# CompVis/stable-diffusion

Measured on AMD Instinct MI355X. Metric: 512x512 images/sec, SD-v1-4 50-step PLMS CFG=7.5, higher is better.
Workload: dtype f16

## Files before the change

### include/sdmi.h

```cpp
#ifndef SDMI_H_
#define SDMI_H_

#include <stdint.h>

#ifdef __cplusplus
extern "C" {
#endif

#define SDMI_ABI_VERSION 17

typedef struct sdmi_unet sdmi_unet;

typedef struct sdmi_unet_cfg {
  int32_t in_channels;
  int32_t out_channels;
  int32_t model_channels;
  int32_t num_res_blocks;
  int32_t n_levels;
  int32_t channel_mult[8];
  int32_t n_attention_resolutions;
  int32_t attention_resolutions[8];
  int32_t num_heads;
  int32_t transformer_depth;
  int32_t context_dim;
// ... 8 lines not shown
#define SDMI_PRECISION_FULL 1
int sdmi_unet_create_with_precision(const sdmi_unet_cfg* cfg, int precision, sdmi_unet** out);
int sdmi_unet_precision(const sdmi_unet* h);
typedef struct sdmi_unet_ext {
  int32_t attention_block;
  int32_t resblock_updown;
} sdmi_unet_ext;
int sdmi_unet_create_ext(const sdmi_unet_cfg* cfg, const sdmi_unet_ext* ext, int precision, sdmi_unet** out);
#define SDMI_UNET_SCALE_SHIFT_NORM 1u
#define SDMI_UNET_NUM_HEAD_CHANNELS_SHIFT 16
#define SDMI_UNET_NUM_HEAD_CHANNELS_MASK 0x0fff0000u
#define SDMI_UNET_NUM_HEAD_CHANNELS(n) (((unsigned)(n) << SDMI_UNET_NUM_HEAD_CHANNELS_SHIFT) & SDMI_UNET_NUM_HEAD_CHANNELS_MASK)
int sdmi_unet_create_flags(const sdmi_unet_cfg* cfg, const sdmi_unet_ext* ext, unsigned flags, int precision, sdmi_unet** out);
int sdmi_unet_destroy(sdmi_unet* h);
int sdmi_unet_num_weights(const sdmi_unet* h);
int sdmi_unet_weight_info(const sdmi_unet* h, int idx, char* key_buf, int key_buf_len, int64_t* shape4, int* ndim);
int sdmi_unet_set_weight(sdmi_unet* h, const char* key, const float* ptr, const int64_t* shape, int ndim, void* stream);
int sdmi_unet_finalize(sdmi_unet* h);

int64_t sdmi_unet_packed_bytes(sdmi_unet* h);
int sdmi_unet_export_packed(sdmi_unet* h, void* host_buf, int64_t bytes, void* stream);
int sdmi_unet_import_packed(sdmi_unet* h, const void* host_buf, int64_t bytes, void* stream);

int64_t sdmi_unet_workspace_bytes(sdmi_unet* h, int B, int H, int W, int Lctx);

int sdmi_unet_cache_context(sdmi_unet* h, const float* ctx, int B, int Lctx, void* workspace, int64_t workspace_bytes,
                            void* stream);
int sdmi_unet_reserve_context(sdmi_unet* h, int B, int Lctx);

int sdmi_unet_cache_timesteps(sdmi_unet* h, const int64_t* t_host, int n, void* stream);
int sdmi_unet_hint_timestep(sdmi_unet* h, int64_t t);
int sdmi_unet_tape_stats(sdmi_unet* h, int64_t* replayed, int64_t* recorded);
int sdmi_unet_skip_fold_plan(sdmi_unet* h, int B, int H, int W, int Lctx, int32_t* folded, int cap);

int sdmi_unet_forward(sdmi_unet* h, const float* x, const int64_t* t_i64, const float* t_f32, const float* ctx,
                      float* eps_out, int B, int H, int W, int Lctx, void* workspace, int64_t workspace_bytes,
                      void* stream);

int sdmi_sampler_step(const float* eps_model, int cfg, float scale, const float* x, int mode, const float* old0,
                      const float* old1, const float* old2, float a_t, float a_prev, float sigma, float sqrt_1m_at,
                      const float* noise, float* e_t_out, float* x_prev, float* pred_x0, int64_t n, void* stream);

int sdmi_sampler_step_x0(const float* eps_model, int cfg, float scale, const float* x, int mode, const float* old0, const float* old1,
                         const float* old2, float a_t, float sqrt_1m_at, float* e_t_out, float* ep_out, float* pred_x0, int64_t n,
                         void* stream);
int sdmi_sampler_step_from_x0(const float* pred_x0, const float* ep, float a_prev, float sigma, const float* noise, float* x_prev,
                              int64_t n, void* stream);

int sdmi_ddpm_step(const float* eps, const float* x0_in, const float* x, float c_recip, float c_recipm1, int clip, float coef1,
                   float coef2, float s, const float* noise, const float* mask, const float* x0_orig, const float* q_noise, float sa,
                   float s1ma, float* x0_out, float* x_prev, int64_t n, void* stream);


int sdmi_dpm_solver_step(const float* eps_model, int cfg, float scale, const float* x, const float* m_prev, float alpha_s,
                         float sigma_s, float cx, float a, float inv_r0, int order, float* m_out, float* x_next, int64_t n,
                         void* stream);

typedef struct sdmi_vae sdmi_vae;
typedef struct sdmi_vae_cfg {
  int32_t ch;
  int32_t out_ch;
  int32_t n_levels;
  int32_t ch_mult[8];
  int32_t num_res_blocks;
  int32_t in_channels;
  int32_t z_channels;
// ... 124 lines not shown

typedef struct sdmi_igemm_desc {
  const void* a0; const void* a1; const void* a2;
  int32_t c0, c1, c2, lda0, lda1, lda2;
  int32_t B, Hin, Win, Hout, Wout, ksize, stride, up;
  const void* w;
  int32_t N;
  int32_t mode;
  const float* bias; const float* rowvec; int32_t ld_rowvec;
  const float* residual; int32_t ldr;
  float* out_f32; void* out_f16; int32_t ldo;
  void* seg_dst[3]; int32_t seg_kind[3];
  int32_t heads, dh, ntok, ntok_pad, segC;
  int32_t splitk;
  float* splitk_ws; int64_t splitk_ws_floats;
  int32_t tile;
  int32_t dma;
  int32_t asym_pad;
  int32_t gn_n; void* gn_acc[2]; int32_t gn_cpg[2]; int32_t gn_cbase[2];
  int32_t* splitk_cnt; int32_t splitk_cnt_ints;
  int32_t split16;
  const float* f16_scale; float* lnp_out;
  const float* lnf_part; int32_t lnf_npart; float lnf_eps; const float* lnf_cs; const float* lnf_d;
  const float* pgn_gamma; const float* pgn_beta; float pgn_eps; int32_t pgn_silu;
  void* pgn_out; int32_t pgn_keep_f32; int32_t* pgn_applied;
  void* out_lo;
} sdmi_igemm_desc;
int sdmi_k_igemm(const sdmi_igemm_desc* d, void* stream);
int sdmi_k_igemm_tail(const sdmi_igemm_desc* d, const void* t0, const void* t1, const void* t2, int tail_c, int tail_ld, const void* tail_w,
                      int tail_kt, void* stream);
int sdmi_k_tail_split_range(int nkt, int nsplit, int split, int* begin, int* end);
int sdmi_k_igemm_up_phase(const sdmi_igemm_desc* d, void* stream);
int sdmi_k_up_phase_weights(const void* w_packed_f16, void* dst_f16, int N, int Cin, void* stream);
int sdmi_k_ff_tail(const sdmi_igemm_desc* proj_out, const void* ln_f16, const float* lnp, float ln_eps, const float* csd,
                   const void* wgg_f16, const void* wff2_f16, const float* bff2, const float* t, void* stream);
int sdmi_k_st_tail(const sdmi_igemm_desc* proj_out, const void* a_f16, const void* wo_f16, const float* bo, float* t, const float* ln_gamma,
                   float ln_eps, const float* csd, const void* wgg_f16, const void* wff2_f16, const float* bff2, void* stream);
int sdmi_k_gn_conv3(const sdmi_igemm_desc* conv, const float* x0, const float* x1, int c0, int c1, float* gn_ws, int64_t gn_ws_floats,
                    const float* gn_gamma, const float* gn_beta, float gn_eps, void* stream);
int sdmi_k_st_head(const float* x, float* gn_ws, int64_t gn_ws_floats, const float* gn_gamma, const float* gn_beta, float gn_eps,
                   const void* w_in3, const float* b_in, float* t, const float* ln_gamma, float ln_eps, const void* wqkv_f16,
                   const float* lnf_cs, const float* lnf_d, void* q, void* k, void* vt, int B, int ntok, int ntok_pad, int heads, int dh,
                   int C, void* stream);
int sdmi_k_st_mid(const void* a_f16, const void* wo_f16, const float* bo, float* t, const float* ln_gamma, float ln_eps, const void* wq_f16,
                  const float* lnf_cs, const float* lnf_d, void* q, int B, int ntok, int heads, int dh, int C, void* stream);
int sdmi_k_st_mid_ctx(const void* a_f16, const void* wo_f16, const float* bo, float* t, const float* ln_gamma, float ln_eps, const void* wq_f16,
                      const float* lnf_cs, const float* lnf_d, const void* ctx_k, const void* ctx_vt, int nkv, int nkv_pad, float scale, void* ao_out,
                      int B, int ntok, int heads, int dh, int C, void* stream);
int sdmi_k_ln_fold_prep(const void* w_f16, int N, int K, int ldw, const float* gamma, const float* beta, const float* bias,
                        float* cs, float* d, void* stream);
int sdmi_k_attention(const void* q, const void* k, const void* vt, void* out, int BH, int heads, int nq, int nkv,
                     int nkv_pad, int d, float scale, void* stream);
int sdmi_k_attention_split16(const void* q, const void* q_lo, const void* k, const void* k_lo, const void* vt, const void* vt_lo, void* out,
                             void* out_lo, int BH, int heads, int nq, int nkv, int nkv_pad, int d, float scale, void* stream);
int sdmi_k_attention_split16_causal(const void* q, const void* q_lo, const void* k, const void* k_lo, const void* vt, const void* vt_lo,
                                    void* out, void* out_lo, int BH, int heads, int n, int n_pad, int d, float scale, void* stream);
int sdmi_k_attention_causal(const void* q, const void* k, const void* vt, void* out, int BH, int heads, int n, int n_pad,
                            int d, float scale, void* stream);
int sdmi_k_groupnorm(const float* x0, const float* x1, int c0, int c1, int B, int HW, const float* gamma,
                     const float* beta, float eps, int silu, void* out_f16, float* out_f32, void* raw_f16, void* out_lo,
                     void* raw_lo, float* partial_ws, int64_t partial_floats, void* stream);
int64_t sdmi_k_groupnorm_ws_floats(int B, int HW);
int sdmi_k_groupnorm_film(const float* x0, const float* x1, int c0, int c1, int B, int HW, const float* gamma, const float* beta, float eps,
                          int silu, const float* film, int film_ld, void* out_f16, float* out_f32, void* raw_f16, void* out_lo, void* raw_lo,
                          float* partial_ws, int64_t partial_floats, void* stream);
int sdmi_k_layernorm(const float* x, const float* gamma, const float* beta, void* out_f16, int M, int C, float eps,
// ... 57 lines not shown
```

### stable-diffusion_amd/_lib.py

```python
import ctypes as C
import os

_HERE = os.path.dirname(os.path.abspath(__file__))
LIB_PATH = os.environ.get('SDMI_LIB_PATH') or os.path.join(_HERE, 'libsdmi.so')

c_f32p = C.c_void_p
c_ptr = C.c_void_p


class UNetCfg(C.Structure):
    _fields_ = [('in_channels', C.c_int32), ('out_channels', C.c_int32), ('model_channels', C.c_int32),
                ('num_res_blocks', C.c_int32), ('n_levels', C.c_int32), ('channel_mult', C.c_int32 * 8),
                ('n_attention_resolutions', C.c_int32), ('attention_resolutions', C.c_int32 * 8),
                ('num_heads', C.c_int32), ('transformer_depth', C.c_int32), ('context_dim', C.c_int32)]


class VaeCfg(C.Structure):
    _fields_ = [('ch', C.c_int32), ('out_ch', C.c_int32), ('n_levels', C.c_int32), ('ch_mult', C.c_int32 * 8),
                ('num_res_blocks', C.c_int32), ('in_channels', C.c_int32), ('z_channels', C.c_int32),
                ('embed_dim', C.c_int32)]


class UNetExt(C.Structure):
    _fields_ = [('attention_block', C.c_int32), ('resblock_updown', C.c_int32)]
# ... 122 lines not shown
    'sdmi_vit_create': (C.c_int, [C.POINTER(VitCfg), C.POINTER(c_ptr)]),
    'sdmi_vit_destroy': (C.c_int, [c_ptr]),
    'sdmi_vit_num_weights': (C.c_int, [c_ptr]),
    'sdmi_vit_weight_info': (C.c_int, [c_ptr, C.c_int, C.c_char_p, C.c_int, C.POINTER(C.c_int64), C.POINTER(C.c_int)]),
    'sdmi_vit_set_weight': (C.c_int, [c_ptr, C.c_char_p, c_ptr, C.POINTER(C.c_int64), C.c_int, c_ptr]),
    'sdmi_vit_finalize': (C.c_int, [c_ptr]),
    'sdmi_vit_workspace_bytes': (C.c_int64, [c_ptr, C.c_int]),
    'sdmi_vit_forward': (C.c_int, [c_ptr, c_ptr, c_ptr, c_ptr, c_ptr, C.c_int, c_ptr, C.c_int64, c_ptr]),
    'sdmi_k_vit_kpad': (C.c_int, [C.c_int]),
    'sdmi_k_vit_patchify': (C.c_int, [c_ptr, c_ptr, C.c_int, C.c_int, C.c_int, c_ptr]),
    'sdmi_k_vit_embed': (C.c_int, [c_ptr, c_ptr, c_ptr, c_ptr, C.c_int, C.c_int, C.c_int, c_ptr]),
    'sdmi_k_vit_preprocess': (C.c_int, [c_ptr, c_ptr, C.c_int, C.c_int, C.c_int, C.c_int, c_ptr]),
    'sdmi_k_safety_head': (C.c_int, [c_ptr, c_ptr, c_ptr, c_ptr, c_ptr, c_ptr, c_ptr, c_ptr, C.c_int, C.c_int, C.c_int, C.c_int, c_ptr]),
    'sdmi_knn_create': (C.c_int, [C.c_int, C.c_int64, C.POINTER(c_ptr)]),
    'sdmi_knn_destroy': (C.c_int, [c_ptr]),
    'sdmi_knn_set_rows': (C.c_int, [c_ptr, C.c_int64, C.c_int64, c_ptr, c_ptr]),
    'sdmi_knn_finalize': (C.c_int, [c_ptr, c_ptr]),
    'sdmi_knn_rows': (C.c_int64, [c_ptr]),
    'sdmi_knn_dim': (C.c_int, [c_ptr]),
    'sdmi_knn_workspace_bytes': (C.c_int64, [c_ptr, C.c_int, C.c_int]),
    'sdmi_knn_search': (C.c_int, [c_ptr, c_ptr, C.c_int, C.c_int, c_ptr, c_ptr, c_ptr, c_ptr, C.c_int64, c_ptr]),
    'sdmi_knn_condition': (C.c_int, [c_ptr, c_ptr, C.c_int, C.c_int, c_ptr, c_ptr, c_ptr, c_ptr, C.c_int64, c_ptr]),
    'sdmi_k_knn_inv_norm': (C.c_int, [c_ptr, C.c_int64, C.c_int, c_ptr, c_ptr]),
    'sdmi_k_knn_scan': (C.c_int, [c_ptr, c_ptr, C.c_int64, C.c_int, c_ptr, C.c_int, C.c_int, C.c_int64, c_ptr, c_ptr, c_ptr]),
    'sdmi_k_knn_merge': (C.c_int, [c_ptr, c_ptr, C.c_int, C.c_int, C.c_int, c_ptr, c_ptr, c_ptr]),
    'sdmi_k_knn_stream_read': (C.c_int, [c_ptr, C.c_int64, c_ptr, c_ptr]),
    'sdmi_k_knn_gather': (C.c_int, [c_ptr, c_ptr, C.c_int64, C.c_int, c_ptr, C.c_int, C.c_int, c_ptr, c_ptr, C.c_int64, c_ptr]),
    'sdmi_has_experiments': (C.c_int, []),
    'sdmi_k_igemm': (C.c_int, [C.POINTER(IGemmDesc), c_ptr]),
    'sdmi_k_igemm_tail': (C.c_int, [C.POINTER(IGemmDesc), c_ptr, c_ptr, c_ptr, C.c_int, C.c_int, c_ptr, C.c_int, c_ptr]),
    'sdmi_k_tail_split_range': (C.c_int, [C.c_int, C.c_int, C.c_int, C.POINTER(C.c_int), C.POINTER(C.c_int)]),
    'sdmi_k_igemm_up_phase': (C.c_int, [C.POINTER(IGemmDesc), c_ptr]),
    'sdmi_k_up_phase_weights': (C.c_int, [c_ptr, c_ptr, C.c_int, C.c_int, c_ptr]),
    'sdmi_tune_lookup': (C.c_int, [C.c_int] * 9 + [C.POINTER(C.c_int), C.POINTER(C.c_int)]),
    'sdmi_unet_skip_fold_plan': (C.c_int, [c_ptr, C.c_int, C.c_int, C.c_int, C.c_int, C.POINTER(C.c_int32), C.c_int]),
    'sdmi_k_ff_tail': (C.c_int, [C.POINTER(IGemmDesc), c_ptr, c_ptr, C.c_float, c_ptr, c_ptr, c_ptr, c_ptr, c_ptr, c_ptr]),
    'sdmi_k_gn_conv3': (C.c_int, [C.POINTER(IGemmDesc), c_ptr, c_ptr, C.c_int, C.c_int, c_ptr, C.c_int64, c_ptr, c_ptr, C.c_float, c_ptr]),
    'sdmi_k_st_mid_ctx': (C.c_int, [c_ptr, c_ptr, c_ptr, c_ptr, c_ptr, C.c_float, c_ptr, c_ptr, c_ptr, c_ptr, c_ptr, C.c_int, C.c_int, C.c_float, c_ptr,
                                    C.c_int, C.c_int, C.c_int, C.c_int, C.c_int, c_ptr]),
    'sdmi_k_st_tail': (C.c_int, [C.POINTER(IGemmDesc), c_ptr, c_ptr, c_ptr, c_ptr, c_ptr, C.c_float, c_ptr, c_ptr, c_ptr, c_ptr, c_ptr]),
    'sdmi_k_st_mid': (C.c_int, [c_ptr, c_ptr, c_ptr, c_ptr, c_ptr, C.c_float, c_ptr, c_ptr, c_ptr, c_ptr, C.c_int, C.c_int, C.c_int, C.c_int,
                                C.c_int, c_ptr]),
    'sdmi_k_st_head': (C.c_int, [c_ptr, c_ptr, C.c_int64, c_ptr, c_ptr, C.c_float, c_ptr, c_ptr, c_ptr, c_ptr, C.c_float, c_ptr, c_ptr, c_ptr,
                                 c_ptr, c_ptr, c_ptr, C.c_int, C.c_int, C.c_int, C.c_int, C.c_int, C.c_int, c_ptr]),
    'sdmi_k_attention_split16': (C.c_int, [c_ptr, c_ptr, c_ptr, c_ptr, c_ptr, c_ptr, c_ptr, c_ptr, C.c_int, C.c_int, C.c_int, C.c_int,
                                           C.c_int, C.c_int, C.c_float, c_ptr]),
    'sdmi_k_attention_split16_causal': (C.c_int, [c_ptr, c_ptr, c_ptr, c_ptr, c_ptr, c_ptr, c_ptr, c_ptr, C.c_int, C.c_int, C.c_int, C.c_int,
                                                  C.c_int, C.c_float, c_ptr]),
    'sdmi_k_attention_causal': (C.c_int, [c_ptr, c_ptr, c_ptr, c_ptr, C.c_int, C.c_int, C.c_int, C.c_int, C.c_int, C.c_float,
                                          c_ptr]),
    'sdmi_k_pointwise_nchw': (C.c_int, [c_ptr, c_ptr, c_ptr, c_ptr, C.c_int, C.c_int, C.c_int, C.c_int, C.c_float, c_ptr]),
    'sdmi_k_softmax_rows': (C.c_int, [c_ptr, c_ptr, C.c_int, C.c_int, C.c_float, c_ptr]),
    'sdmi_k_gelu_erf': (C.c_int, [c_ptr, c_ptr, C.c_int64, c_ptr]),
    'sdmi_k_quick_gelu': (C.c_int, [c_ptr, c_ptr, C.c_int64, c_ptr]),
    'sdmi_k_quick_gelu_split': (C.c_int, [c_ptr, c_ptr, c_ptr, C.c_int64, c_ptr]),
    'sdmi_k_gelu_erf_split': (C.c_int, [c_ptr, c_ptr, c_ptr, C.c_int64, c_ptr]),
    'sdmi_k_attention': (C.c_int, [c_ptr, c_ptr, c_ptr, c_ptr, C.c_int, C.c_int, C.c_int, C.c_int, C.c_int, C.c_int,
                                   C.c_float, c_ptr]),
    'sdmi_k_groupnorm': (C.c_int, [c_ptr, c_ptr, C.c_int, C.c_int, C.c_int, C.c_int, c_ptr, c_ptr, C.c_float, C.c_int,
                                   c_ptr, c_ptr, c_ptr, c_ptr, c_ptr, c_ptr, C.c_int64, c_ptr]),
    'sdmi_k_groupnorm_ws_floats': (C.c_int64, [C.c_int, C.c_int]),
    'sdmi_k_groupnorm_film': (C.c_int, [c_ptr, c_ptr, C.c_int, C.c_int, C.c_int, C.c_int, c_ptr, c_ptr, C.c_float, C.c_int, c_ptr, C.c_int,
                                        c_ptr, c_ptr, c_ptr, c_ptr, c_ptr, c_ptr, C.c_int64, c_ptr]),
    'sdmi_k_layernorm': (C.c_int, [c_ptr, c_ptr, c_ptr, c_ptr, C.c_int, C.c_int, C.c_float, c_ptr]),
    'sdmi_k_cast_f16': (C.c_int, [c_ptr, c_ptr, c_ptr, C.c_int64, c_ptr]),
    'sdmi_k_split_heads': (C.c_int, [c_ptr, C.c_int, C.c_int, c_ptr, c_ptr, C.c_int, C.c_int, C.c_int, C.c_int, C.c_int, C.c_int,
# ... 70 lines not shown
```

### stable-diffusion_amd/build.py

```python
import concurrent.futures as cf
import hashlib
import os
import subprocess
import sys

HERE = os.path.dirname(os.path.abspath(__file__))
CSRC = os.path.join(HERE, 'csrc')
EXTRA = os.environ.get('SDMI_CXXFLAGS', '').split()
LIB = os.path.join(HERE, os.environ.get('SDMI_LIB_OUT', 'libsdmi.so'))
OBJ = os.path.join(HERE, 'build' if os.path.basename(LIB) == 'libsdmi.so' else 'build_' + os.path.splitext(os.path.basename(LIB))[0])
SOURCES = ['igemm_t1.hip', 'igemm_t0.hip', 'igemm_t2.hip', 'igemm_h1.hip', 'igemm_h0.hip', 'igemm_h2.hip', 'igemm.hip', 'conv3halo.hip', 'gemm_split16.hip', 'rowchain.hip', 'gnconv.hip', 'range.hip', 'attn.hip', 'attn_wide.hip', 'attn_split16.hip', 'attn_wide_split16.hip', 'split_ops.hip', 'norm.hip', 'small.hip', 'sampler.hip', 'inpaint.hip', 'patch.hip', 'vit.hip', 'knn.hip', 'textpool.hip', 'rescale.hip', 'weights.cpp', 'unet.cpp', 'vae.cpp', 'clip.cpp', 'bert.cpp', 'api.cpp', 'prof.cpp']
FLAGS = ['--offload-arch=gfx950', '-O3', '-std=c++17', '-fPIC', '-munsafe-fp-atomics', '-Wall', '-Wno-unused-function',
         '-Wno-unused-variable']


def _hipcc():
    for c in (os.environ.get('HIPCC'), '/opt/rocm/bin/hipcc', 'hipcc'):
        if c and (not os.path.isabs(c) or os.path.exists(c)):
            return c
    raise RuntimeError('hipcc not found')


def _stamp():
    h = hashlib.sha256()
    for root in (CSRC, os.path.join(os.path.dirname(HERE), 'include')):
        for fn in sorted(os.listdir(root)):
            with open(os.path.join(root, fn), 'rb') as f:
                h.update(fn.encode())
                h.update(f.read())
    h.update(' '.join(FLAGS + EXTRA).encode())
    return h.hexdigest()


def is_current():
    stamp_file = os.path.join(OBJ, 'stamp')
    return os.path.exists(LIB) and os.path.exists(stamp_file) and open(stamp_file).read() == _stamp()


def build(force=False, verbose=True):
    os.makedirs(OBJ, exist_ok=True)
    stamp_file = os.path.join(OBJ, 'stamp')
    if not force and is_current():
        return LIB
    hipcc = _hipcc()
# ... 56 lines not shown
```

### stable-diffusion_amd/csrc/api.cpp

```cpp
#include <string.h>

#include <new>

#include "prof.h"
#include "split16.h"
#include "unet.h"
#include "vae.h"
#include "clip.h"
#include "knn.h"
#include "rescale.h"

namespace sdmi {
static thread_local std::string g_err;
void set_error(const std::string& msg) { g_err = msg; }
int fail(const std::string& msg) { g_err = msg; return -1; }
}

struct sdmi_unet { sdmi::UNet impl; };
struct sdmi_vae { sdmi::Vae impl; };
struct sdmi_clip { sdmi::ClipText impl; };
struct sdmi_bert { sdmi::BertText impl; };
struct sdmi_vit { sdmi::ClipVision impl; };
struct sdmi_knn { sdmi::Knn impl; };

// ... 523 lines not shown
  p.pgn_gamma = d->pgn_gamma; p.pgn_beta = d->pgn_beta; p.pgn_eps = d->pgn_eps; p.pgn_silu = d->pgn_silu;
  p.pgn_out = (f16*)d->pgn_out; p.pgn_keep_f32 = d->pgn_keep_f32; p.pgn_applied = d->pgn_applied;
  p.out_lo = (f16*)d->out_lo;
  return zero_page(&p.zero_page);
}
int sdmi_k_igemm(const sdmi_igemm_desc* d, void* stream) {
  SDMI_CHECK(d, "null descriptor");
  IGemmParams p = IGemmParams();
  if (igemm_params_of(d, p)) return -1;
  IGemmTune t; t.tile = d->tile; t.dma = d->dma;
  return launch_igemm(p, t, (hipStream_t)stream);
}
int sdmi_k_igemm_tail(const sdmi_igemm_desc* d, const void* t0, const void* t1, const void* t2, int tail_c, int tail_ld, const void* tail_w,
                      int tail_kt, void* stream) {
  SDMI_CHECK(d, "null descriptor");
  IGemmParams p = IGemmParams();
  if (igemm_params_of(d, p)) return -1;
  p.tail_a0 = (const f16*)t0; p.tail_a1 = (const f16*)t1; p.tail_a2 = (const f16*)t2;
  p.tail_c = tail_c; p.tail_ld = tail_ld; p.tail_w = (const f16*)tail_w; p.tail_kt = tail_kt;
  IGemmTune t; t.tile = d->tile; t.dma = d->dma;
  return launch_igemm(p, t, (hipStream_t)stream);
}
int sdmi_k_igemm_up_phase(const sdmi_igemm_desc* d, void* stream) {
  SDMI_CHECK(d, "null descriptor");
  IGemmParams p = IGemmParams();
  if (igemm_params_of(d, p)) return -1;
  SDMI_CHECK(p.ksize == 3 && p.up == 1 && p.stride == 1 && p.Hout == 2 * p.Hin && p.Wout == 2 * p.Win && p.c1 == 0 && p.c2 == 0 && !p.split16,
             "up_phase: the descriptor is the reference op, a 3x3 stride-1 conv of one nearest-x2 upsampled source (Hout = 2 Hin, Wout = 2 Win)");
  IGemmParams q = up_phase_of(p, p.w);
  q.splitk = d->splitk;
  IGemmTune t; t.tile = d->tile; t.dma = d->dma;
  return launch_igemm(q, t, (hipStream_t)stream);
}
int sdmi_k_up_phase_weights(const void* w_packed, void* dst, int N, int Cin, void* stream) {
  return launch_up_phase_weights((const f16*)w_packed, (f16*)dst, N, Cin, (hipStream_t)stream);
}
int sdmi_k_tail_split_range(int nkt, int nsplit, int split, int* begin, int* end) {
  SDMI_CHECK(begin && end && nkt >= 0 && nsplit >= 1 && split >= 0 && split < nsplit, "bad arguments");
  tail_split_range(nkt, nsplit, split, begin, end);
  return 0;
}
int sdmi_tune_lookup(int M, int N, int K, int ksize, int stride, int up, int mode, int splitk_req, int kt, int* tile, int* splitk) {
  SDMI_CHECK(tile && splitk, "null argument");
  return tune_lookup(M, N, K, ksize, stride, up, mode, splitk_req, kt, tile, splitk);
}
int sdmi_unet_skip_fold_plan(sdmi_unet* h, int B, int H, int W, int Lctx, int32_t* folded, int cap) {
  SDMI_CHECK(h && (folded || cap == 0), "null argument");
  int64_t need = 0;
  if (h->impl.run(nullptr, nullptr, nullptr, nullptr, nullptr, B, H, W, Lctx, nullptr, 0, nullptr, true, false, &need)) return -1;
  const std::vector<int>& plan = h->impl.skip_fold_plan_;
  for (int i = 0; i < (int)plan.size() && i < cap; ++i) folded[i] = plan[i];
  return (int)plan.size();
}
int sdmi_k_ff_tail(const sdmi_igemm_desc* proj_out, const void* ln_f16, const float* lnp, float ln_eps, const float* csd,
                   const void* wgg_f16, const void* wff2_f16, const float* bff2, const float* t, void* stream) {
  SDMI_CHECK(proj_out, "null descriptor");
  FfTailParams q = FfTailParams();
  if (igemm_params_of(proj_out, q.epi)) return -1;
  SDMI_CHECK(proj_out->split16 && proj_out->ksize == 1, "ff_tail: the proj_out descriptor is a split-fp16 1x1 (w = sdmi_k_pack_split3)");
  q.ln = (const f16*)ln_f16; q.lnp = lnp; q.ln_eps = ln_eps; q.csd = csd; q.wgg = (const f16*)wgg_f16; q.wff2 = (const f16*)wff2_f16;
  q.bff2 = bff2; q.t = t; q.wpo = (const f16*)proj_out->w;
  return launch_ff_tail(q, (hipStream_t)stream);
}
int sdmi_k_st_tail(const sdmi_igemm_desc* proj_out, const void* a_f16, const void* wo_f16, const float* bo, float* t, const float* ln_gamma,
                   float ln_eps, const float* csd, const void* wgg_f16, const void* wff2_f16, const float* bff2, void* stream) {
  SDMI_CHECK(proj_out && a_f16, "null argument");
  FfTailParams q = FfTailParams();
  if (igemm_params_of(proj_out, q.epi)) return -1;
  SDMI_CHECK(proj_out->split16 && proj_out->ksize == 1, "st_tail: the proj_out descriptor is a split-fp16 1x1 (w = sdmi_k_pack_split3)");
  q.a16 = (const f16*)a_f16; q.wo = (const f16*)wo_f16; q.bo = bo; q.ln_gamma = ln_gamma; q.ln_eps = ln_eps; q.csd = csd;
  q.wgg = (const f16*)wgg_f16; q.wff2 = (const f16*)wff2_f16; q.bff2 = bff2; q.t = t; q.wpo = (const f16*)proj_out->w;
  return launch_ff_tail(q, (hipStream_t)stream);
}
int sdmi_k_gn_conv3(const sdmi_igemm_desc* conv, const float* x0, const float* x1, int c0, int c1, float* gn_ws, int64_t gn_ws_floats,
                    const float* gn_gamma, const float* gn_beta, float gn_eps, void* stream) {
  SDMI_CHECK(conv && x0 && gn_ws && gn_gamma && gn_beta, "gn_conv3: null argument");
  GnConvParams q = GnConvParams();
  if (igemm_params_of(conv, q.epi)) return -1;
  const int B = q.epi.B;
  SDMI_CHECK(gn_ws_floats >= gn_acc_words(B) * 2, "groupnorm workspace too small");
  SDMI_HIP_OK(hipMemsetAsync(gn_ws, 0, gn_acc_words(B) * sizeof(long long), (hipStream_t)stream));
  GroupNormParams g = GroupNormParams();
  g.x0 = x0; g.c0 = c0; g.x1 = x1; g.c1 = c1; g.B = B; g.HW = q.epi.Hout * q.epi.Wout; g.gamma = gn_gamma; g.beta = gn_beta; g.eps = gn_eps;
// ... 185 lines not shown
```

### stable-diffusion_amd/csrc/common.h

```cpp
#pragma once
#include <hip/hip_runtime.h>
#include <stdint.h>
#include <algorithm>
#include <string>

#include "tape.h"

typedef _Float16 f16;
typedef _Float16 f16x2 __attribute__((ext_vector_type(2)));
typedef _Float16 f16x4 __attribute__((ext_vector_type(4)));
typedef _Float16 f16x8 __attribute__((ext_vector_type(8)));
typedef float f32x4 __attribute__((ext_vector_type(4)));
typedef float f32x16 __attribute__((ext_vector_type(16)));

#ifdef __HIPCC__
__device__ __forceinline__ float gn_apply_elem(float v, float mean, float rstd, float gamma, float beta, int silu) {
  float t = __builtin_fmaf((v - mean) * rstd, gamma, beta);
  if (silu) t = t * __builtin_amdgcn_rcpf(1.0f + __expf(-t));
  return t;
}
__device__ __forceinline__ float gn_apply_film_elem(float v, float mean, float rstd, float gamma, float beta, float scale, float shift,
                                                    int silu) {
  float t = __builtin_fmaf((v - mean) * rstd, gamma, beta);
  t = __builtin_fmaf(t, 1.0f + scale, shift);
// ... 15 lines not shown
  *hi = (long long)h;
  *lo = __double2ll_rn((d - h) * 1099511627776.0);
}
__device__ __forceinline__ void gn_mean_rstd(long long s, long long sl, long long ss, long long ssl, double n, float eps,
                                             float* mean, float* rstd) {
  const double m = gn_acc_value(s, sl) / n;
  double var = gn_acc_value(ss, ssl) / n - m * m;
  if (var < 0.0) var = 0.0;
  *mean = (float)m;
  *rstd = (float)(1.0 / sqrt(var + (double)eps));
}
#endif

namespace sdmi {

void set_error(const std::string& msg);
int fail(const std::string& msg);

#define SDMI_HIP_OK(expr)                                                                    \
  do {                                                                                       \
    hipError_t _e = (expr);                                                                  \
    if (_e != hipSuccess)                                                                    \
      return ::sdmi::fail(std::string(#expr) + ": " + hipGetErrorString(_e));                \
  } while (0)

#define SDMI_CHECK(cond, msg)                                                                \
  do {                                                                                       \
    if (!(cond)) return ::sdmi::fail(std::string("check failed: ") + #cond + " -- " + (msg)); \
  } while (0)

static inline int cdiv(int a, int b) { return (a + b - 1) / b; }
static inline int64_t round_up(int64_t a, int64_t b) { return (a + b - 1) / b * b; }

enum EpiMode { EPI_PLAIN = 0, EPI_GEGLU = 1, EPI_HEADS = 2 };

#ifdef SDMI_NT_STORES
#define SDMI_ST(T, ptr, val) __builtin_nontemporal_store((T)(val), (T*)(ptr))
#else
#define SDMI_ST(T, ptr, val) (*(T*)(ptr) = (T)(val))
#endif
#ifndef SDMI_W_AUX
#define SDMI_W_AUX 0
#endif
#ifndef SDMI_WT_STORES
#define SDMI_WT_STORES 1
#endif
#if defined(__HIPCC__) && SDMI_WT_STORES >= 1
typedef unsigned sdmi_u32x4 __attribute__((ext_vector_type(4)));
typedef unsigned sdmi_u32x2 __attribute__((ext_vector_type(2)));
__device__ __forceinline__ void sdmi_st_wt16(const void* base, size_t byte_off, f32x4 v) {
  if (__builtin_expect(byte_off < (size_t)0x80000000u - 16, 1)) {
    const __amdgpu_buffer_rsrc_t r = __builtin_amdgcn_make_buffer_rsrc((void*)base, 0, (int)0x80000000, 0x00020000);
    __builtin_amdgcn_raw_buffer_store_b128(__builtin_bit_cast(sdmi_u32x4, v), r, (int)byte_off, 0, 16);
  } else {
    *(f32x4*)((char*)base + byte_off) = v;
  }
}
__device__ __forceinline__ void sdmi_st_wt8(const void* base, size_t byte_off, f16x4 v) {
  if (__builtin_expect(byte_off < (size_t)0x80000000u - 16, 1)) {
    const __amdgpu_buffer_rsrc_t r = __builtin_amdgcn_make_buffer_rsrc((void*)base, 0, (int)0x80000000, 0x00020000);
    __builtin_amdgcn_raw_buffer_store_b64(__builtin_bit_cast(sdmi_u32x2, v), r, (int)byte_off, 0, 16);
  } else {
    *(f16x4*)((char*)base + byte_off) = v;
  }
}
#define SDMI_ST_F32X4(base, off, val) sdmi_st_wt16((base), (size_t)(off) * 4, (val))
#if SDMI_WT_STORES >= 2
// ... 39 lines not shown
  int nkt = 0;
#ifdef SDMI_IGEMM_TIMING
  long long* dbg_times = nullptr;
  int dbg_abl = 0;
#endif
  int splitk_fused = 0;
  int slab_tiled = 0, slab_bm = 0, slab_bn = 0, slab_wm = 0, slab_wn = 0;
  int slab_sh_qpt = 0, slab_sh_nt = 0, slab_sh_tn = 0, slab_sh_wn = 0;
  int epi_vec = 0;
  int tile_n_fastest = 0;
  const f16* zero_page = nullptr;
  int gn_n = 0;
  long long* gn_acc[2] = {nullptr, nullptr};
  int gn_cpg[2] = {0, 0}, gn_cbase[2] = {0, 0};
  unsigned long long gn_magic[2] = {0, 0};
  const float* pgn_gamma = nullptr; const float* pgn_beta = nullptr; float pgn_eps = 1e-5f; int pgn_silu = 1;
  f16* pgn_out = nullptr;
  int pgn_keep_f32 = 0;
  int* pgn_applied = nullptr;
  unsigned long long magic_hw = 0, magic_w = 0, magic_w2 = 0;
  int log2w = 0;
  const float* xf0 = nullptr; const float* xf1 = nullptr;
  const long long* gn_in_acc = nullptr;
  const float* gn_in_gamma = nullptr; const float* gn_in_beta = nullptr; float gn_in_eps = 1e-5f; int gn_in_silu = 1;
  f16* raw_hi = nullptr; f16* raw_lo = nullptr;
  f16* gn_scratch = nullptr;
  unsigned long long magic_cpg_in = 0;
  int halo_thi = 0, halo_ipt = 1, log2_tpi = 30;
  unsigned long long magic_hpi = 0;
  const f16* tail_a0 = nullptr; const f16* tail_a1 = nullptr; const f16* tail_a2 = nullptr;
  int tail_c = 0, tail_ld = 0;
  const f16* tail_w = nullptr;
  int tail_kt = 0;
};
__host__ __device__ static inline void tail_split_range(int nkt, int nsplit, int split, int* begin, int* end) {
  *begin = (int)(((long long)split * nkt) / nsplit);
  *end = (int)(((long long)(split + 1) * nkt) / nsplit);
}

constexpr int SDMI_NUM_TILES = 22;
struct IGemmTune {
  int tile = -1;
  int dma = -1;
};

int launch_igemm(const IGemmParams& p, const IGemmTune& tune, hipStream_t stream);
bool igemm_plans_halo(const IGemmParams& p);
bool igemm_plans_up_phase(const IGemmParams& p);
static inline IGemmParams up_phase_of(const IGemmParams& p, const f16* w_phase) {
  IGemmParams q = p;
  q.ksize = 2; q.Hout = p.Hin; q.Wout = p.Win; q.M = p.B * p.Hin * p.Win; q.K = 4 * p.c0; q.w = w_phase; q.splitk = 0;
  return q;
}
int tune_lookup(int M, int N, int K, int ksize, int stride, int up, int mode, int splitk_req, int kt, int* tile, int* splitk);
bool range_check_enabled();
uint64_t tune_generation();
bool tune_collecting();
int range_check_set(int enable);
int range_scan(const char* what, const f16* p, int64_t n, hipStream_t stream);
int range_report(std::string* json);

int tune_begin();
int tune_round(int r);
int tune_end(const char* path, int* n_keys);
int tune_dump(std::string* out);
int launch_splitk_reduce(const IGemmParams& p, int nsplit, hipStream_t stream);
// ... 40 lines not shown
  long long* dbg = nullptr;
#endif
};
bool st_head_supported(int C, int M, int ntok, int ntok_pad, int heads, int dh);
int launch_st_head(const StHeadParams& p, hipStream_t stream);
int launch_st_mid(const StHeadParams& p, hipStream_t stream);

struct GnConvParams {
  const float* x0 = nullptr; const float* x1 = nullptr; int c0 = 0, c1 = 0;
  const long long* gn_acc = nullptr;
  const float* gn_gamma = nullptr; const float* gn_beta = nullptr; float gn_eps = 1e-5f;
  const f16* w = nullptr;
#ifdef SDMI_RC_TIMING
  long long* dbg = nullptr;
#endif
  IGemmParams epi;
};
bool gn_conv3_supported(int B, int H, int W, int c0, int c1, int Cout);
int launch_gn_conv3(const GnConvParams& p, hipStream_t stream);

struct AttnParams {
  const f16* q = nullptr;
  const f16* k = nullptr;
  const f16* vt = nullptr;
  f16* out = nullptr;
  int BH = 0, heads = 0, nq = 0, nkv = 0, nkv_pad = 0, d = 0;
  float scale = 1.f;
  int nw = 0;
  int causal = 0;
  int prio = 0;
  int pingpong = 0;
};
int launch_attention(const AttnParams& p, hipStream_t stream);
int launch_attention_wide(const AttnParams& p, hipStream_t stream);

struct GroupNormParams {
  const float* x0 = nullptr; const float* x1 = nullptr; int c0 = 0, c1 = 0;
  int B = 0, HW = 0;
  const float* gamma = nullptr; const float* beta = nullptr; float eps = 1e-5f;
  int silu = 0;
  int stats_only = 0;
  int skip_stats = 0;
  f16* out_f16 = nullptr;
  float* out_f32 = nullptr;
  f16* raw_f16 = nullptr;
  f16* out_lo = nullptr;
  f16* raw_lo = nullptr;
  const float* film = nullptr; int film_ld = 0;
  long long* acc = nullptr;
};
constexpr int GN_SLOTS = 8;
constexpr int GN_MAX_CALLS = 96;
constexpr int GN_WORDS = 4;
constexpr int GN_STRIDE = 16;
static inline int64_t gn_acc_words(int B) { return (int64_t)B * 32 * GN_SLOTS * GN_STRIDE; }
int launch_groupnorm(const GroupNormParams& p, hipStream_t stream);

int launch_layernorm(const float* x, const float* gamma, const float* beta, f16* out, int M, int C, float eps,
                     hipStream_t stream, float* out_f32 = nullptr);
int launch_cast_f16(const float* x, f16* out, f16* out_lo, int64_t n, hipStream_t stream);

int launch_timestep_embedding(const int64_t* t_i64, const float* t_f32, float* out, int B, int dim, hipStream_t s);
int launch_small_linear(const float* in, int ld_in, const float* w, const float* bias, float* out, int ld_out,
                        int B, int N, int K, int silu_in, hipStream_t s);
int launch_ctx1_broadcast(const f16* vt, int ld_v, f16* ao, int B, int ntok, int C, hipStream_t s);
int launch_conv_in(const float* x_nchw, const float* w, const float* bias, float* out_nhwc, int B, int Cin, int H,
// ... 98 lines not shown
```

### stable-diffusion_amd/csrc/igemm.hip

```cpp
#include <dlfcn.h>

#include <map>
#include <mutex>
#include <tuple>
#include <vector>

#include "igemm_dev.h"

namespace sdmi {
namespace {

__global__ void __launch_bounds__(256) splitk_reduce_kernel(IGemmParams p, int nsplit, int rows_per_block) {
  __shared__ unsigned long long s_gn[2][32][GN_WORDS];
  const int tx = threadIdx.x & 7, ty = threadIdx.x >> 3;
  const int n = (blockIdx.x * 8 + tx) * 4;
  const int row0 = blockIdx.y * rows_per_block;
  const int HW = p.Hout * p.Wout;
  const bool gn = p.gn_n > 0;
  const bool ncol = n < p.N;
  if (gn) {
    for (int i = threadIdx.x; i < 2 * 32 * GN_WORDS; i += 256) (&s_gn[0][0][0])[i] = 0ull;
    __syncthreads();
  }
  const size_t slab_sz = (size_t)p.M * p.N;
// ... 343 lines not shown
  SDMI_HIP_OK(hipGetLastError());
  ps2.end();
  if (p.ln_out) return launch_layernorm(p.out_f32, p.ln_gamma, p.ln_beta, p.ln_out, p.M, p.N, p.ln_eps, stream);
  return 0;
}

struct TileCfg { int bm, bn, wm, wn, ns; };
static const TileCfg kTiles[SDMI_NUM_TILES] = {
    {128, 128, 2, 2, 2},
    {128, 64, 2, 2, 2},
    {64, 64, 2, 2, 2},
    {256, 128, 4, 2, 2},
    {128, 64, 2, 2, 3},
    {64, 64, 2, 2, 3},
    {256, 128, 4, 2, 3},
    {128, 128, 2, 2, 3},
    {64, 128, 2, 2, 3},
    {128, 128, 4, 2, 3},
    {64, 64, 2, 2, 4},
    {128, 256, 2, 4, 2},
    {64, 256, 1, 4, 3},
    {256, 64, 4, 1, 3},
    {256, 64, 4, 2, 5},
    {256, 128, 4, 2, 3},
    {128, 64, 2, 2, 8},
    {128, 128, 2, 2, 5},
    {64, 64, 2, 2, 8},
    {64, 128, 2, 2, 6},
    {128, 64, 2, 2, 6},
    {128, 128, 4, 2, 4},
};
static inline bool tile_is_halo(int t) { return t >= 14 && t <= 17; }
static inline bool tile_tn_even(int t) { return (kTiles[t].bn / kTiles[t].wn / 32) % 2 == 0; }

static int launch_tile(int tile, const IGemmParams& p, bool dma, int splitk, hipStream_t stream) {
  if (p.tail_kt && !tile_is_halo(tile)) return fail("a GEMM with a 1x1 tail phase was routed to tile " + std::to_string(tile) + ": only the halo-staged conv tiles 14..17 run a tail");
  if (p.split16) return launch_split16_tile(tile, p, splitk, stream);
  if (igemm_has_half(p)) {
    switch (tile) {
      case 0: case 1: case 2: case 3: case 4: case 5: return launch_generic_tile_h0(tile, p, dma, splitk, stream);
      case 6: case 7: case 8: case 9: case 10: return launch_generic_tile_h1(tile, p, dma, splitk, stream);
      case 11: case 12: case 13: case 18: case 19: case 20: case 21: return launch_generic_tile_h2(tile, p, dma, splitk, stream);
      default: break;
    }
  }
  switch (tile) {
    case 0: case 1: case 2: case 3: case 4: case 5: return launch_generic_tile_g0(tile, p, dma, splitk, stream);
    case 6: case 7: case 8: case 9: case 10: return launch_generic_tile_g1(tile, p, dma, splitk, stream);
    case 11: case 12: case 13: case 18: case 19: case 20: case 21: return launch_generic_tile_g2(tile, p, dma, splitk, stream);
    case 14: case 15: case 16: case 17: return launch_halo_tile(tile, p, splitk, stream);
    default: return fail("unknown igemm tile id");
  }
}

struct TuneKey {
  int M, N, K, ksize, stride, up, mode, splitk_req;
  int kt = 0;
  bool operator<(const TuneKey& o) const {
    return std::tie(M, N, K, ksize, stride, up, mode, splitk_req, kt) <
           std::tie(o.M, o.N, o.K, o.ksize, o.stride, o.up, o.mode, o.splitk_req, o.kt);
  }
};
struct TuneChoice { int tile, splitk; double us; };
struct TuneRec { TuneKey key; int cand; hipEvent_t e0, e1; };

class Tuner {
 public:
  std::mutex mu;
  std::map<TuneKey, TuneChoice> table;
  bool loaded = false, collecting = false;
  int round = 0;
  std::vector<TuneRec> recs;
  std::map<TuneKey, std::vector<std::pair<TuneChoice, std::vector<float>>>> stats;
  std::vector<hipEvent_t> pool;

  static std::string default_path() {
    if (const char* e = getenv("SDMI_TUNE_FILE")) return e;
    Dl_info info;
    if (dladdr((const void*)&Tuner::default_path, &info) && info.dli_fname) {
      std::string so = info.dli_fname;
      const size_t k = so.find_last_of('/');
      return (k == std::string::npos ? std::string(".") : so.substr(0, k)) + "/tune_gfx950.txt";
    }
    return "tune_gfx950.txt";
  }
  static std::string phase_path_of(const std::string& table_path) {
    static const std::string base = "tune_gfx950.txt";
    if (table_path.size() >= base.size() && table_path.compare(table_path.size() - base.size(), base.size(), base) == 0)
      return table_path.substr(0, table_path.size() - base.size()) + "tune_up_phase_gfx950.txt";
    return table_path + ".up_phase";
  }
  void load_file(const std::string& path) {
    FILE* f = fopen(path.c_str(), "r");
    if (!f) return;
    char line[256];
    while (fgets(line, sizeof line, f)) {
      if (line[0] == '#') continue;
      TuneKey k; TuneChoice c; c.us = 0;
      k.kt = 0;
      if (sscanf(line, "%d %d %d %d %d %d %d %d %d %d %lf %d", &k.M, &k.N, &k.K, &k.ksize, &k.stride, &k.up, &k.mode,
                 &k.splitk_req, &c.tile, &c.splitk, &c.us, &k.kt) >= 10 && c.tile >= 0 && c.tile < SDMI_NUM_TILES && c.splitk >= 1 &&
          c.splitk <= 16 && k.kt >= 0)
        table[k] = c;
    }
    fclose(f);
  }
  void ensure_loaded() {
    if (loaded) return;
    loaded = true;
    if (env_int("SDMI_TUNE_DISABLE", 0)) return;
    load_file(default_path());
    load_file(phase_path_of(default_path()));
  }
  std::map<TuneKey, TuneChoice>::const_iterator find_entry(TuneKey k) const {
    auto it = table.find(k);
    if (it == table.end() && k.kt) { k.kt = 0; it = table.find(k); }
    return it;
  }
  hipEvent_t ev() {
    if (!pool.empty()) { hipEvent_t e = pool.back(); pool.pop_back(); return e; }
    hipEvent_t e = nullptr;
    (void)hipEventCreate(&e);
    return e;
  }
};
static Tuner g_tuner;

static std::vector<TuneChoice> tune_candidates(const IGemmParams& p, bool can_split) {
  std::vector<TuneChoice> out;
  const int nkt = igemm_nkt(p);
  static const int splits[] = {1, 2, 3, 4, 5, 6, 8, 10, 12, 16};
  for (int t = 0; t < SDMI_NUM_TILES; ++t) {
    const TileCfg& c = kTiles[t];
    if (tile_is_halo(t) && !halo_supported(p, c.bm)) continue;
    if (p.tail_kt && !tile_is_halo(t)) continue;
    if (p.split16 && !split16_tile_supported(t)) continue;
    if (!p.split16 && ((c.ns == 2 && t != 11 && !tile_is_halo(t)) || t == 12 || t == 13)) continue;
    if (p.mode == EPI_GEGLU && !tile_tn_even(t)) continue;
    if (p.lnp_out && (p.M % c.bm || p.N % c.bn || (p.Hout * p.Wout) % c.bm)) continue;
    const long blocks = (long)cdiv(p.M, c.bm) * cdiv(p.N, c.bn);
    if ((long)c.bm > 2L * p.M && c.bm > 64) continue;
    if ((long)c.bn > 2L * p.N && c.bn > 64) continue;
    for (int sk : splits) {
      if ((sk == 5 || sk == 10) && !tile_is_halo(t)) continue;
      if (sk > 1) {
        if (p.splitk != 0 || !can_split || p.ksize == 2) break;
        if (nkt / sk < 4) break;
        if (tile_is_halo(t) && (nkt / 9) % sk != 0) continue;
        if (blocks * (sk / 2 + 1) > 1536) break;
        if (splitk_ws_need(p, c.bm, c.bn, sk) > p.splitk_ws_floats) break;
      }
      if (blocks * sk < 48 && sk < 16 && nkt / (sk * 2) >= 4 && can_split && p.splitk == 0 && p.ksize != 2) continue;
      out.push_back({t, p.splitk > 1 ? p.splitk : sk, 0.0});
      if (p.splitk != 0) break;
    }
  }
  if (out.empty()) out.push_back({5, p.splitk > 0 ? p.splitk : 1, 0.0});
  return out;
}

int tune_begin() {
  std::lock_guard<std::mutex> lk(g_tuner.mu);
  g_tuner.ensure_loaded();
  g_tuner.collecting = true; g_tuner.round = 0;
  g_tuner.recs.clear(); g_tuner.stats.clear();
  return 0;
}
int tune_round(int r) {
  std::lock_guard<std::mutex> lk(g_tuner.mu);
  g_tuner.round = r;
  return 0;
}
static int tune_drain() {
  for (auto& r : g_tuner.recs) {
    float ms = 0.f;
    SDMI_HIP_OK(hipEventSynchronize(r.e1));
    SDMI_HIP_OK(hipEventElapsedTime(&ms, r.e0, r.e1));
    auto& v = g_tuner.stats[r.key];
    if ((int)v.size() > r.cand) v[r.cand].second.push_back(ms * 1e3f);
    g_tuner.pool.push_back(r.e0); g_tuner.pool.push_back(r.e1);
  }
  g_tuner.recs.clear();
  return 0;
}
bool tune_collecting() { return g_tuner.collecting; }
static uint64_t g_tune_generation = 0;
uint64_t tune_generation() { return g_tune_generation; }
int tune_end(const char* path, int* n_keys) {
  std::lock_guard<std::mutex> lk(g_tuner.mu);
  if (!g_tuner.collecting) return fail("sdmi_tune_end without sdmi_tune_begin");
  if (tune_drain()) return -1;
  g_tuner.collecting = false;
  auto score = [](std::vector<float> v) -> double {
    if (v.empty()) return 1e30;
    std::sort(v.begin(), v.end());
    return v.size() % 2 ? v[v.size() / 2] : 0.5 * (v[v.size() / 2 - 1] + v[v.size() / 2]);
  };
  for (auto& kv : g_tuner.stats) {
    double best = 1e30; const TuneChoice* bc = nullptr;
    for (auto& c : kv.second) {
      const double sc = score(c.second);
      if (sc < best) { best = sc; bc = &c.first; }
    }
    if (bc) g_tuner.table[kv.first] = {bc->tile, bc->splitk, best};
  }
  if (n_keys) *n_keys = (int)g_tuner.stats.size();
  ++g_tune_generation;
  const std::string out = (path && *path) ? std::string(path) : Tuner::default_path();
  bool any_phase = false;
  for (auto& kv : g_tuner.table) any_phase = any_phase || kv.first.ksize == 2;
  for (int which = 0; which < (any_phase ? 2 : 1); ++which) {
    const std::string path_w = which ? Tuner::phase_path_of(out) : out;
    FILE* f = fopen(path_w.c_str(), "w");
    if (!f) return fail("cannot write the tuning table to " + path_w);
    fputs(which ? "# libsdmi igemm tuning table (gfx950), the 2x2 phase convs of the Upsample convs (ksize 2: M = rows of one phase, K = 4 Cin; compared with "
                       "the site's up = 1 row of the main table), measured in situ by tools/tune.py -- M N K ksize stride up mode splitk_req tile splitk us\n"
                     : "# libsdmi igemm tuning table (gfx950), measured in situ by tools/tune.py -- M N K ksize stride up mode splitk_req tile splitk us\n", f);
    for (auto& kv : g_tuner.table) {
      const TuneKey& k = kv.first;
      if ((k.ksize == 2) != (which == 1)) continue;
      fprintf(f, "%d %d %d %d %d %d %d %d %d %d %.2f", k.M, k.N, k.K, k.ksize, k.stride, k.up, k.mode, k.splitk_req, kv.second.tile,
              kv.second.splitk, kv.second.us);
      if (k.kt) fprintf(f, " %d", k.kt);
      fprintf(f, "\n");
    }
    fclose(f);
  }
  return 0;
}
int tune_dump(std::string* out) {
  std::lock_guard<std::mutex> lk(g_tuner.mu);
  char buf[256];
  for (auto& kv : g_tuner.stats) {
    const TuneKey& k = kv.first;
    for (auto& c : kv.second) {
      if (c.second.empty()) continue;
      std::vector<float> v = c.second;
      std::sort(v.begin(), v.end());
      snprintf(buf, sizeof buf, "%d %d %d %d %d %d %d %d%s | %d %d %.2f %.2f %d\n", k.M, k.N, k.K, k.ksize, k.stride, k.up, k.mode,
               k.splitk_req, k.kt ? (" t" + std::to_string(k.kt)).c_str() : "", c.first.tile, c.first.splitk, (double)v[v.size() / 2], (double)v[0], (int)v.size());
      *out += buf;
    }
  }
  return 0;
}

int tune_lookup(int M, int N, int K, int ksize, int stride, int up, int mode, int splitk_req, int kt, int* tile, int* splitk) {
  std::lock_guard<std::mutex> lk(g_tuner.mu);
  g_tuner.ensure_loaded();
  auto it = g_tuner.find_entry(TuneKey{M, N, K, ksize, stride, up, mode, splitk_req, kt});
  if (it == g_tuner.table.end()) return 1;
  *tile = it->second.tile; *splitk = it->second.splitk;
  return 0;
// ... 44 lines not shown
               "upsample phase convs: nearest x2 of one source of whole 64-channel chunks (Hout x Wout = the SOURCE map), plain epilogue without residual / "
               "LayerNorm / tail, unsplit");
  const int Cin = p.c0 + p.c1 + p.c2;
  SDMI_CHECK(p.K == p.ksize * p.ksize * Cin, "K != ksize^2 * (c0 + c1 + c2)");
  SDMI_CHECK(p.c0 % BKH == 0 && p.c1 % BKH == 0 && p.c2 % BKH == 0 && p.c0 > 0, "channel counts of every A source must be multiples of 32");
  SDMI_CHECK((p.c2 == 0 || p.c1 > 0), "third A source without a second");
  SDMI_CHECK(p.lda0 % 8 == 0 && (p.a1 == nullptr || p.lda1 % 8 == 0), "A row pitch must be a multiple of 8 halves");
  SDMI_CHECK(p.zero_page != nullptr, "zero page missing");
  SDMI_CHECK(p.M == p.B * p.Hout * p.Wout, "M != B * Hout * Wout");
  SDMI_CHECK(p.c1 == 0 || p.a1 != nullptr, "second A source missing");
  SDMI_CHECK(p.c2 == 0 || (p.a2 != nullptr && p.lda2 % 8 == 0), "third A source missing");
  SDMI_CHECK((p.c1 == 0 || p.lda1 == p.lda0) && (p.c2 == 0 || p.lda2 == p.lda0), "all A sources must share one row pitch");
  SDMI_CHECK(!p.up || ((p.ksize == 3 || phase) && p.stride == 1), "upsample folding needs a 3x3 stride-1 conv");
  if (p.mode == EPI_GEGLU) SDMI_CHECK(p.N % 64 == 0 && p.out_f16 != nullptr, "GEGLU needs N % 64 == 0 and an fp16 output");
  if (p.ln_out)
    SDMI_CHECK(p.mode == EPI_PLAIN && p.out_f32 && p.ldo == p.N && p.N % 4 == 0 && p.N <= 2560 && p.ln_gamma && p.ln_beta,
               "LayerNorm post-op needs plain mode, an fp32 output with ldo == N <= 2560, gamma and beta");
  if (p.out_lo) SDMI_CHECK(p.mode == EPI_PLAIN && p.ldo % 4 == 0, "out_lo needs plain mode");
  if (p.lnp_out || p.f16_scale)
    SDMI_CHECK(p.mode == EPI_PLAIN && p.out_f32 && p.out_f16 && !p.out_lo && !p.ln_out && p.N % 64 == 0 && p.M % 64 == 0 &&
                   (p.Hout * p.Wout) % 64 == 0 && p.splitk == 1 && epi_vec_ok(p),
               "LayerNorm row statistics: plain mode, fp32 + fp16 outputs, no split-K, M / N / rows per sample multiples of 64, 16-byte aligned rows");
  if (p.lnf_part)
    SDMI_CHECK(p.ksize == 1 && p.c1 == 0 && p.c2 == 0 && !p.split16 && p.lnf_npart * 32 == p.K && p.lnf_cs && p.lnf_d && !p.bias &&
                   p.splitk == 1 && p.lnf_npart <= 40,
               "LayerNorm-folding GEMM: dense, one source, K = 32 * lnf_npart <= 1280, column sums + offsets, no bias, no split-K");
  if (p.gn_n) {
    SDMI_CHECK(p.mode == EPI_PLAIN && p.gn_n <= 2 && (p.Hout * p.Wout) % 32 == 0, "GroupNorm statistics need plain mode and Hout*Wout % 32 == 0");
    SDMI_CHECK(p.N % 4 == 0, "GroupNorm statistics: N % 4 == 0");
    for (int t = 0; t < p.gn_n; ++t)
      SDMI_CHECK(p.gn_acc[t] && p.gn_cpg[t] >= 2 && (p.gn_cbase[t] + p.N + p.gn_cpg[t] - 1) / p.gn_cpg[t] <= 32, "bad GroupNorm statistics target");
  }
  if (p.mode == EPI_HEADS) SDMI_CHECK(p.segC > 0 && p.dh > 0 && p.N % p.segC == 0 && p.N / p.segC <= 3, "bad head scatter");

  SDMI_CHECK((int64_t)p.B * p.Hin * p.Win * p.lda0 * 2 + (int64_t)(p.Win + 1) * p.lda0 * 2 < ((int64_t)1 << 31) - 65536 &&
                 (int64_t)p.N * p.K * 2 < ((int64_t)1 << 31) - 65536,
             "tensor too large for 31-bit byte offsets (buffer addressing)");
  static const int env_dma = env_int("SDMI_IGEMM_DMA", 1);
  static const int env_tile = env_int("SDMI_IGEMM_TILE", -1);
  const bool dma = (tune.dma >= 0 ? tune.dma : env_dma) != 0;
  int tile = tune.tile >= 0 ? tune.tile : env_tile;
  SDMI_CHECK(tile < SDMI_NUM_TILES, "unknown igemm tile id");
  int splitk = p.splitk;
  const int nkt = igemm_nkt(p);
  static const int env_split = env_int("SDMI_SPLITK", -1);
  const bool can_split_plain = p.mode == EPI_PLAIN && p.splitk_ws && p.N % 4 == 0 && p.ldo % 4 == 0 &&
                               (p.residual == nullptr || p.ldr % 4 == 0);
  const bool can_split_heads = p.mode == EPI_HEADS && p.splitk_ws && p.dh % 4 == 0 && p.segC % 4 == 0;
  const bool can_split = can_split_plain || can_split_heads;
  if (env_split >= 0 && splitk == 0 && !phase) splitk = env_split;

  hipEvent_t ev0 = nullptr, ev1 = nullptr;
  TuneKey tkey{p.M, p.N, nkt * BK, p.split16 ? 11 : p.ksize, p.stride, p.up, p.mode, splitk, p.tail_kt};
  int tcand = -1;
  if (tile < 0) {
    std::lock_guard<std::mutex> lk(g_tuner.mu);
    g_tuner.ensure_loaded();
    static const int only_ksize = env_int("SDMI_TUNE_ONLY_KSIZE", -1);
    if (g_tuner.collecting && (only_ksize < 0 || tkey.ksize == only_ksize)) {
      IGemmParams q = p; q.splitk = splitk;
      const std::vector<TuneChoice> cands = tune_candidates(q, can_split);
      auto& st = g_tuner.stats[tkey];
      if (st.empty()) for (auto& c : cands) st.push_back({c, {}});
      tcand = g_tuner.round % (int)cands.size();
      tile = cands[tcand].tile; splitk = cands[tcand].splitk;
      ev0 = g_tuner.ev(); ev1 = g_tuner.ev();
    } else {
      auto it = g_tuner.find_entry(tkey);
      if (it != g_tuner.table.end()) {
        const int tt = it->second.tile, sk = it->second.splitk;
        const bool halo = tile_is_halo(tt);
        const bool ws_ok = sk == 1 || (can_split && splitk_ws_need(p, kTiles[tt].bm, kTiles[tt].bn, sk) <= p.splitk_ws_floats);
        const bool split_ok = splitk != 0 ? (sk == splitk && ws_ok)
                                          : (sk == 1 || (ws_ok && nkt / sk >= 4 && (halo || (sk != 5 && sk != 10)) &&
                                                         (!halo || (nkt / 9) % sk == 0)));
        if (split_ok && (p.mode != EPI_GEGLU || tile_tn_even(tt)) && (!halo || halo_supported(p, kTiles[tt].bm)) &&
            (!p.split16 || split16_tile_supported(tt)) && (!phase || sk == 1)) {
          tile = tt; splitk = sk;
        }
      }
    }
  }
  if (p.mode == EPI_GEGLU && tile >= 0 && !tile_tn_even(tile)) tile = 0;
  if (p.split16) {
    if (tile >= 0) SDMI_CHECK(split16_tile_supported(tile), "split-fp16 GEMM: tile id without an instantiation");
    else tile = 5;
  }
  if (tile < 0) {
    const double gflop = 2.0 * p.M * (double)p.N * p.K * 1e-9;
    if (p.mode == EPI_GEGLU) tile = 0;
    else if (p.mode == EPI_HEADS) tile = 2;
    else tile = gflop >= 25.0 ? 3 : 5;
  }
  if (p.lnp_out) {
    const int hw = p.Hout * p.Wout;
    if (p.M % kTiles[tile].bm || p.N % kTiles[tile].bn || hw % kTiles[tile].bm || (p.split16 && !split16_tile_supported(tile))) tile = 5;
  }
  if (phase) {
    SDMI_CHECK(!tile_is_halo(tile) && splitk <= 1, "upsample phase convs run unsplit on the generic tiles");
    splitk = 1;
  }
  if (splitk <= 0) {
    splitk = 1;
    if (can_split) {
      const long blocks = (long)cdiv(p.M, kTiles[tile].bm) * cdiv(p.N, kTiles[tile].bn);
      const long want = (kTiles[tile].wm * kTiles[tile].wn == 8) ? 160 : 512;
      while (blocks * splitk < want && nkt / (splitk * 2) >= 8 && splitk < 16 &&
             splitk_ws_need(p, kTiles[tile].bm, kTiles[tile].bn, splitk * 2) <= p.splitk_ws_floats)
        splitk *= 2;
    }
  }
  if (splitk > 1) {
    SDMI_CHECK(can_split, "split-K needs plain or head-scatter mode, a slab workspace and N / ldo / ldr multiples of 4");
    SDMI_CHECK(splitk_ws_need(p, kTiles[tile].bm, kTiles[tile].bn, splitk) <= p.splitk_ws_floats, "split-K workspace too small");
  }
  if (ev0) SDMI_HIP_OK(hipEventRecord(ev0, stream));
#ifdef SDMI_IGEMM_TIMING
  static const char* dbg_path = getenv("SDMI_IGEMM_TIMING");
  static const int dbg_abl = env_int("SDMI_EPI_ABL", 0);
  static long long* dbg_buf = nullptr;
  constexpr int DBG_WG = 16384;
  IGemmParams pd = p;
  pd.dbg_abl = dbg_abl;
  if (dbg_path) {
    if (!dbg_buf) SDMI_HIP_OK(hipMalloc((void**)&dbg_buf, 6 * DBG_WG * sizeof(long long)));
    SDMI_HIP_OK(hipMemsetAsync(dbg_buf, 0, 6 * DBG_WG * sizeof(long long), stream));
// ... 56 lines not shown
```

### stable-diffusion_amd/csrc/igemm_dev.h

```cpp
#pragma once
#include "common.h"
#include "prof.h"

namespace sdmi {
typedef unsigned u32x4 __attribute__((ext_vector_type(4)));

int launch_splitk_reduce(const IGemmParams& p, int nsplit, hipStream_t stream);
int launch_generic_tile_g0(int tile, const IGemmParams& p, bool dma, int splitk, hipStream_t stream);
int launch_generic_tile_g1(int tile, const IGemmParams& p, bool dma, int splitk, hipStream_t stream);
int launch_generic_tile_g2(int tile, const IGemmParams& p, bool dma, int splitk, hipStream_t stream);
int launch_generic_tile_h0(int tile, const IGemmParams& p, bool dma, int splitk, hipStream_t stream);
int launch_generic_tile_h1(int tile, const IGemmParams& p, bool dma, int splitk, hipStream_t stream);
int launch_generic_tile_h2(int tile, const IGemmParams& p, bool dma, int splitk, hipStream_t stream);

static int env_int(const char* name, int dflt) {
  const char* v = getenv(name);
  return v ? atoi(v) : dflt;
}

namespace {

constexpr int BK = 64;
constexpr int BKH = 32;
static inline int src_chunks(int c) { return (c + BK - 1) / BK; }
// ... 78 lines not shown
#pragma unroll
    for (int r = 0; r < 16; ++r) a[j][r] = wl[((r & 3) + 8 * (r >> 2) + 4 * lg) * LSTR + j * 32 + l31];
  asm volatile("s_waitcnt lgkmcnt(0)" ::: "memory");
}

constexpr int LNF_MAXP = 40;
__device__ __forceinline__ void lnf_request(const IGemmParams& p, int m, float2 (&pv)[LNF_MAXP]) {
  const float2* src = (const float2*)p.lnf_part + m;
#pragma unroll
  for (int j = 0; j < 20; ++j) pv[j] = src[(size_t)min(j, p.lnf_npart - 1) * p.M];
  if (p.lnf_npart > 20) {
#pragma unroll
    for (int j = 20; j < LNF_MAXP; ++j) pv[j] = src[(size_t)min(j, p.lnf_npart - 1) * p.M];
  } else {
#pragma unroll
    for (int j = 20; j < LNF_MAXP; ++j) pv[j] = float2{0.f, 0.f};
  }
}
__device__ __forceinline__ void lnf_finish(const IGemmParams& p, const float2 (&pv)[LNF_MAXP], float* mean, float* rstd) {
  float s = 0.f, q = 0.f;
#pragma unroll
  for (int j = 0; j < LNF_MAXP; ++j)
    if (j < p.lnf_npart) { s += pv[j].x; q += pv[j].y; }
  const float inv_c = 1.0f / (32.0f * (float)p.lnf_npart);
  const float mu = s * inv_c;
  const float var = fmaxf(q * inv_c - mu * mu, 0.f);
  *mean = mu;
  *rstd = 1.0f / sqrtf(var + p.lnf_eps);
}
__device__ __forceinline__ float sum8_dpp(float v) {
  v += __builtin_bit_cast(float, __builtin_amdgcn_update_dpp(0, __builtin_bit_cast(int, v), 0xB1, 0xF, 0xF, true));
  v += __builtin_bit_cast(float, __builtin_amdgcn_update_dpp(0, __builtin_bit_cast(int, v), 0x4E, 0xF, 0xF, true));
  v += __builtin_bit_cast(float, __builtin_amdgcn_update_dpp(0, __builtin_bit_cast(int, v), 0x141, 0xF, 0xF, true));
  return v;
}

template <int BM, int BN, int WARPS_M, int WARPS_N, int LDS_BYTES, bool PHASE = false>
__device__ __forceinline__ void igemm_epilogue(const IGemmParams& p_arg, f32x16 (&acc)[BM / WARPS_M / 32][BN / WARPS_N / 32],
                                               const int m0, const int n0, const int split, const int tile_m,
                                               const int tile_n, unsigned char* smem, const float lnf_mean = 0.f,
                                               const float lnf_rstd = 1.f, const int phase = 0) {
#ifdef SDMI_IGEMM_TIMING
  IGemmParams p = p_arg;
  if (p.dbg_abl & 1) p.residual = nullptr;
  if (p.dbg_abl & 4) { p.out_f32 = nullptr; p.out_f16 = nullptr; p.out_lo = nullptr; }
#else
  const IGemmParams& p = p_arg;
#endif
  constexpr int NT = WARPS_M * WARPS_N * 64;
  constexpr int WTM = BM / WARPS_M, WTN = BN / WARPS_N;
  constexpr int TM = WTM / 32, TN = WTN / 32;
  constexpr int LSTR = SLAB_LSTR<WARPS_M * WARPS_N, WTN, LDS_BYTES>;
  const int tid = threadIdx.x;
  const int lane = tid & 63;
  const int wave = tid >> 6;
  const int wm = wave / WARPS_N, wn = wave - wm * WARPS_N;
  const int l31 = lane & 31, lg = lane >> 5;
  const int HWout = p.Hout * p.Wout;
  auto orow = [&](int m) -> size_t {
    if constexpr (PHASE) {
      const int b = fast_div_hw(m, p.magic_hw);
      const int rem = m - b * HWout;
      const int i = fast_div(rem, p.magic_w), j = rem - i * p.Wout;
      return ((size_t)(b * 2 * p.Hout + 2 * i + (phase >> 1)) * (size_t)(2 * p.Wout) + (size_t)(2 * j + (phase & 1)));
    } else {
      return (size_t)m;
// ... 48 lines not shown
#pragma unroll
            for (int j = 0; j < TN; ++j)
#pragma unroll
              for (int r4 = 0; r4 < 4; ++r4)
#pragma unroll
                for (int e = 0; e < 4; ++e) acc[i][j][4 * r4 + e] += v[ss][(i * TN + j) * 4 + r4][e];
        }
      }
    }
    __syncthreads();
  }
  if (p.splitk > 1 && !p.splitk_fused && p.slab_tiled) {
    constexpr int SC1 = 16;
    const int tiles_n_all = (p.N + BN - 1) / BN, ntiles = ((p.M + BM - 1) / BM) * tiles_n_all;
    const int tile_lin = tile_m * tiles_n_all + tile_n;
    const __amdgpu_buffer_rsrc_t ws = __builtin_amdgcn_make_buffer_rsrc(
        (void*)(p.splitk_ws + ((size_t)split * ntiles + tile_lin) * (size_t)(BM * BN)), 0, BM * BN * 4, 0x00020000);
#pragma unroll
    for (int i = 0; i < TM; ++i)
#pragma unroll
      for (int j = 0; j < TN; ++j)
#pragma unroll
        for (int r4 = 0; r4 < 4; ++r4) {
          const f32x4 v = {acc[i][j][4 * r4], acc[i][j][4 * r4 + 1], acc[i][j][4 * r4 + 2], acc[i][j][4 * r4 + 3]};
          __builtin_amdgcn_raw_buffer_store_b128(__builtin_bit_cast(u32x4, v), ws, (tid * 4 + ((i * TN + j) * 4 + r4) * (NT * 4)) * 4, 0, SC1);
        }
    return;
  }
  if (p.lnf_part) {
    __syncthreads();
    float2* const tab = (float2*)smem;
    if (tid < BM) tab[tid] = float2{lnf_mean, lnf_rstd};
    __syncthreads();
#pragma unroll
    for (int j = 0; j < TN; ++j) {
      const int n = min(nw + j * 32 + l31, p.N - 1);
      const float cs = p.lnf_cs[n], dn = p.lnf_d[n];
#pragma unroll
      for (int i = 0; i < TM; ++i)
#pragma unroll
        for (int r = 0; r < 16; ++r) {
          const float2 mr = tab[wm * WTM + i * 32 + (r & 3) + 8 * (r >> 2) + 4 * lg];
          acc[i][j][r] = fmaf(mr.y, acc[i][j][r] - mr.x * cs, dn);
        }
    }
    __syncthreads();
  }
  const bool unfused_split = p.splitk > 1 && !p.splitk_fused;
  if (p.mode == EPI_PLAIN) {
    const bool atomic = unfused_split;
    float* slab = atomic ? (p.splitk_ws + (size_t)split * p.M * p.N) : nullptr;
    const int b_first = m0 / HWout;
    const bool one_batch = ((m0 + BM - 1) / HWout == b_first);
    if (full && one_batch && p.epi_vec && !atomic) {
      __syncthreads();
      float* const wl = slab_base<WARPS_M * WARPS_N, WTN, LDS_BYTES>(smem, wave);
      const int rl = lane / SLAB_LPR<WTN>, c4 = (lane % SLAB_LPR<WTN>) * 4;
      f32x4 colv = {0.f, 0.f, 0.f, 0.f};
      if (p.bias) colv = *(const f32x4*)(p.bias + nw + c4);
      if (p.rowvec) colv += *(const f32x4*)(p.rowvec + (size_t)b_first * p.ld_rowvec + nw + c4);
      f32x4 g4 = {1.f, 1.f, 1.f, 1.f};
      if (p.f16_scale) g4 = *(const f32x4*)(p.f16_scale + nw + c4);
#pragma unroll
      for (int i = 0; i < TM; ++i) {
        slab_put<TN, LSTR>(wl, acc[i], l31, lg);
        constexpr int NP = SLAB_NPASS<WTN>, RPI = SLAB_RPI<WTN>;
        f32x4 resv[NP];
        if (p.residual) {
#pragma unroll
          for (int q = 0; q < NP; ++q)
// ... 176 lines not shown
    }
  } else if (p.mode == EPI_GEGLU) {
    if constexpr (TN % 2 == 0) {
#pragma unroll
      for (int j2 = 0; j2 < TN / 2; ++j2) {
        const int nv = nw + (2 * j2) * 32 + l31;
        if (nv >= p.N) continue;
        const float bv = p.bias ? p.bias[nv] : 0.f, bg = p.bias ? p.bias[nv + 32] : 0.f;
        const int oc = (nw >> 1) + j2 * 32 + l31;
        if (full) {
#pragma unroll
          for (int i = 0; i < TM; ++i)
#pragma unroll
            for (int r = 0; r < 16; ++r) {
              const int m = mw + i * 32 + (r & 3) + 8 * (r >> 2) + 4 * lg;
              const float val = acc[i][2 * j2][r] + bv;
              const float gate = acc[i][2 * j2 + 1][r] + bg;
              SDMI_ST(f16, p.out_f16 + (size_t)m * p.ldo + oc, (f16)(val * gelu_erf(gate)));
            }
        } else {
#pragma unroll
          for (int i = 0; i < TM; ++i)
#pragma unroll
            for (int r = 0; r < 16; ++r) {
              const int m = mw + i * 32 + (r & 3) + 8 * (r >> 2) + 4 * lg;
              if (m >= p.M) continue;
              const float val = acc[i][2 * j2][r] + bv;
              const float gate = acc[i][2 * j2 + 1][r] + bg;
              p.out_f16[(size_t)m * p.ldo + oc] = (f16)(val * gelu_erf(gate));
            }
        }
      }
    }
  } else {
    if (unfused_split) {
      float* slab = p.splitk_ws + (size_t)split * p.M * p.N;
#pragma unroll
      for (int i = 0; i < TM; ++i)
#pragma unroll
        for (int r = 0; r < 16; ++r) {
          const int m = mw + i * 32 + (r & 3) + 8 * (r >> 2) + 4 * lg;
          if (m >= p.M) continue;
#pragma unroll
          for (int j = 0; j < TN; ++j) {
            const int n = nw + j * 32 + l31;
            if (n < p.N) slab[(size_t)m * p.N + n] = acc[i][j][r];
          }
        }
      return;
    }
    if (p.bias) {
#pragma unroll
      for (int j = 0; j < TN; ++j) {
        const int n = nw + j * 32 + l31;
        const float bv = n < p.N ? p.bias[n] : 0.f;
#pragma unroll
        for (int i = 0; i < TM; ++i)
#pragma unroll
          for (int r = 0; r < 16; ++r) acc[i][j][r] += bv;
      }
    }
    const bool vecq = full && p.epi_vec;
    if (vecq) {
      __syncthreads();
      float* const wl = slab_base<WARPS_M * WARPS_N, WTN, LDS_BYTES>(smem, wave);
      const int rl = lane / SLAB_LPR<WTN>, c4 = (lane % SLAB_LPR<WTN>) * 4;
// ... 137 lines not shown
```

### stable-diffusion_amd/csrc/igemm_kernel.h

```cpp
#pragma once
#include <string>

#include "igemm_dev.h"

namespace sdmi {
namespace {


template <int BM, int BN, int WARPS_M, int WARPS_N, bool DMA, int NS, int KIND, bool HALF = false>
__global__ void __launch_bounds__(WARPS_M* WARPS_N * 64) igemm_kernel(const IGemmParams p, const int tiles_m,
                                                                       const int tiles_n, const int kt_per_split) {
  static_assert(DMA || NS == 2, "the register-staged path is double buffered");
#if defined(__HIP_DEVICE_COMPILE__)
  constexpr bool UP = KIND == KIND_3X3_UP;
  constexpr bool K2 = KIND == KIND_2X2;
  constexpr bool K3 = KIND != KIND_1X1;
  constexpr int TW = K2 ? 2 : 3;
  static_assert(!K2 || (DMA && !HALF), "the 2x2 phase kind: LDS-DMA, whole 64-channel chunks");
  constexpr int NT = WARPS_M * WARPS_N * 64;
  constexpr int RPP = NT / 8;
  constexpr int A_PASSES = BM / RPP;
  constexpr int B_PASSES = BN / RPP;
  constexpr int WTM = BM / WARPS_M, WTN = BN / WARPS_N;
  constexpr int TM = WTM / 32, TN = WTN / 32;
// ... 74 lines not shown
          if (iy >= 0 && iy < p.Hin && ix >= 0 && ix < p.Win) mk |= 1u << t;
        }
        a_mask[i] = mk | ((HALF && gch < 4) ? mk << 9 : 0u);
      }
    }
  }
  int b_off[B_PASSES];
#pragma unroll
  for (int i = 0; i < B_PASSES; ++i) {
    const int n = min(n0 + i * RPP + lrow, p.N - 1);
    b_off[i] = (n * p.K + gch * 8) * 2;
  }

  f16x8 regA[DMA ? 1 : A_PASSES], regB[DMA ? 1 : B_PASSES];
  const int wave_u = __builtin_amdgcn_readfirstlane(wave);

  int ld_kt = kt_begin;
  int ld_tap = K3 ? kt_begin % ntap : 0;
  int ld_cin0 = (kt_begin / ntap) * BK;
  int ld_ky = K3 ? ld_tap / TW : 0, ld_kx = K3 ? ld_tap - TW * (ld_tap / TW) : 0;
  const int pc0 = p.c0, pc1 = p.c1, pc2 = p.c2;
  const int pp0 = (pc0 + BK - 1) & ~(BK - 1), pp01 = pp0 + ((pc1 + BK - 1) & ~(BK - 1));
  int ld_boff = 0;
  if constexpr (HALF) {
    const int dense0 = ld_cin0 - (ld_cin0 >= pp0 ? pp0 - pc0 : 0) - (ld_cin0 >= pp01 ? pp01 - pp0 - pc1 : 0);
    const int left = ld_cin0 < pp0 ? pc0 - ld_cin0 : (ld_cin0 < pp01 ? pc1 - (ld_cin0 - pp0) : pc2 - (ld_cin0 - pp01));
    ld_boff = (ntap * dense0 + ld_tap * min(left, BK)) * 2;
  }

  constexpr int OOB = (int)0x80000000;
  const long long a_shift = (K3 && !UP) ? (long long)(pad_y * p.Win + pad_x) * ld * 2 : 0;
  const char* const srcA0 = (const char*)p.a0 - a_shift; const char* const srcA1 = (const char*)p.a1 - a_shift;
  const char* const srcA2 = (const char*)p.a2 - a_shift;
  const f16* const w_base = K2 ? p.w + (size_t)split * (size_t)p.N * (size_t)p.K : p.w;
  const __amdgpu_buffer_rsrc_t rsrc_w = __builtin_amdgcn_make_buffer_rsrc((void*)w_base, 0, OOB, 0x00020000);
  const int pWin = p.Win;

  struct TileCursor { __amdgpu_buffer_rsrc_t rsrc_a; int a_soff, b_soff; unsigned tapbit; int ky, kx; unsigned lds; int half; };
  auto next_tile = [&](int stage) {
    TileCursor c;
    const char* src; int coff, left;
    if (ld_cin0 < pp0) { src = srcA0; coff = ld_cin0; left = pc0 - coff; }
    else if (ld_cin0 < pp01) { src = srcA1; coff = ld_cin0 - pp0; left = pc1 - coff; }
    else { src = srcA2; coff = ld_cin0 - pp01; left = pc2 - coff; }
    const bool half = HALF && left < BK;
    c.rsrc_a = __builtin_amdgcn_make_buffer_rsrc((void*)src, 0, OOB, 0x00020000);
    c.a_soff = ((K3 && !UP) ? (ld_ky * pWin + ld_kx) * ld + coff : coff) * 2;
    c.b_soff = HALF ? ld_boff : ld_kt * (BK * 2);
    c.tapbit = 1u << (half ? ld_tap + 9 : ld_tap); c.ky = ld_ky; c.kx = ld_kx;
    c.half = half ? OOB : 0;
    c.lds = stage * STAGE_BYTES;
    if (ld_kt + 1 < kt_end) {
      ++ld_kt;
      if constexpr (HALF) ld_boff += half ? BKH * 2 : BK * 2;
      if constexpr (K3) {
        ++ld_tap;
        if (++ld_kx == TW) { ld_kx = 0; ++ld_ky; }
        if (ld_tap == ntap) { ld_tap = 0; ld_ky = 0; ld_kx = 0; ld_cin0 += BK; }
      } else {
        ld_cin0 += BK;
      }
    }
    return c;
  };
  auto a_voff = [&](const TileCursor& c, int i) -> int {
    int v;
    if constexpr (UP) v = a_ro[i][c.ky] + a_co[i][c.kx];
// ... 116 lines not shown
      const int cur = (kt - kt_begin) & 1;
      __syncthreads();
      const bool more = (kt + 1 < kt_end);
      if (more) issue_loads(cur ^ 1);
#pragma unroll
      for (int ks = 0; ks < BK / 16; ++ks) {
        f16x8 a[TM], b[TN];
        read_frags(cur, ks, a, b);
        mfma_step(a, b);
      }
      if (more) commit_regs(cur ^ 1);
    }
  }

  SDMI_STAMP(dbg_t2);
  igemm_epilogue<BM, BN, WARPS_M, WARPS_N, NS * STAGE_BYTES, K2>(p, acc, m0, n0, K2 ? 0 : split, tile_m, tile_n, smem, lnf_mean, lnf_rstd,
                                                                 K2 ? split : 0);
#ifdef SDMI_IGEMM_TIMING
  if (p.dbg_times && tid == 0) {
    long long* d = p.dbg_times + 6 * (size_t)blockIdx.x;
    d[0] = dbg_t0; d[1] = dbg_t1; d[2] = dbg_t2; d[4] = (long long)__builtin_readcyclecounter();
  }
#endif
#endif
}

template <int BM, int BN, int WARPS_M, int WARPS_N, int NS, bool HALF = false>
int launch_cfg(const IGemmParams& p, bool dma, int splitk, hipStream_t stream) {
  SDMI_CHECK(HALF || (p.c0 % BK == 0 && p.c1 % BK == 0 && p.c2 % BK == 0), "internal: a half k-tile launch on the whole-chunk kernel");
  const int tiles_m = cdiv(p.M, BM), tiles_n = cdiv(p.N, BN);
  const int nkt = igemm_nkt(p);
  const int kt_per_split = cdiv(nkt, splitk);
  const int nsplit = cdiv(nkt, kt_per_split);
  IGemmParams q = p;
  q.nkt = nkt;
  q.splitk = nsplit;
  q.tile_n_fastest = tile_order_n_fastest(p);
  q.splitk_fused = 0;
  slab_layout(q, BM, BN, WARPS_M, WARPS_N, nsplit);
  q.epi_vec = epi_vec_ok(p);
  SDMI_CHECK(splitk_ws_need(p, BM, BN, nsplit) <= p.splitk_ws_floats, "split-K workspace too small");
  SDMI_CHECK((int64_t)p.M < (int64_t)65536 * p.Hout * p.Wout, "fast_div_hw: at most 65535 samples per launch");
  q.magic_hw = div_magic_hw(p.Hout * p.Wout);
  q.magic_w = div_magic(p.Wout);
  for (int t = 0; t < p.gn_n; ++t) q.gn_magic[t] = div_magic(p.gn_cpg[t]);
  const bool phase = p.ksize == 2;
  if (phase) SDMI_CHECK(!HALF && dma && nsplit == 1, "the 2x2 phase convs run unsplit on the LDS-DMA kernels, whole 64-channel chunks only");
  dim3 grid(tiles_m * tiles_n * (phase ? 4 : nsplit)), block(WARPS_M * WARPS_N * 64);
  static const int by_shape = env_int("SDMI_PROF_SHAPES", 0);
  std::string pname = std::string("igemm_") + std::to_string(BM) + "x" + std::to_string(BN) + "w" +
                      std::to_string(WARPS_M * WARPS_N) + "s" + std::to_string(NS) + (HALF ? "h" : "") + (phase ? "_up2x2" : "");
  if (by_shape && prof_enabled())
    pname += "_M" + std::to_string(p.M) + "_N" + std::to_string(p.N) + "_K" + std::to_string(p.K) + "_k" +
             std::to_string(p.ksize) + "_m" + std::to_string(p.mode) + "_s" + std::to_string(nsplit);
  const double src_pix = (double)p.B * p.Hin * p.Win;
  const double out_b = (p.out_f32 ? 4.0 : 0.0) + ((p.out_f16 || p.mode != EPI_PLAIN) ? 2.0 : 0.0);
  const double n_out = p.mode == EPI_GEGLU ? p.N / 2.0 : (double)p.N;
  const int k_alg = p.k_alg > 0 ? p.k_alg : p.K;
  const double cin_alg = p.k_alg > 0 ? (double)p.k_alg : (double)(p.c0 + p.c1 + p.c2);
  const double m_out = phase ? 4.0 * p.M : (double)p.M;
  const double k_ref = phase ? 9.0 * cin_alg : (double)k_alg;
  ProfScope ps(pname.c_str(), 2.0 * m_out * (double)p.N * k_ref,
               src_pix * cin_alg * 2.0 + (double)p.N * k_ref * 2.0 + m_out * n_out * out_b +
                   (p.residual ? (double)p.M * p.N * 4.0 : 0.0),
               stream, 2.0 * m_out * (double)p.N * p.K);
  const int kind = p.ksize == 1 ? KIND_1X1 : (phase ? KIND_2X2 : (p.up ? KIND_3X3_UP : KIND_3X3));
#define SDMI_LAUNCH_KIND(K_)                                                                                        \
  do {                                                                                                              \
    if (dma) SDMI_LAUNCH((igemm_kernel<BM, BN, WARPS_M, WARPS_N, true, NS, K_, HALF>), grid, block, 0, stream, q,   \
                                tiles_m, tiles_n, kt_per_split);                                                    \
    else SDMI_LAUNCH((igemm_kernel<BM, BN, WARPS_M, WARPS_N, false, 2, K_, HALF>), grid, block, 0, stream, q,       \
                            tiles_m, tiles_n, kt_per_split);                                                        \
  } while (0)
  if (kind == KIND_1X1) SDMI_LAUNCH_KIND(KIND_1X1);
  else if (kind == KIND_3X3) SDMI_LAUNCH_KIND(KIND_3X3);
  else if (kind == KIND_3X3_UP) SDMI_LAUNCH_KIND(KIND_3X3_UP);
  else if constexpr (!HALF) SDMI_LAUNCH((igemm_kernel<BM, BN, WARPS_M, WARPS_N, true, NS, KIND_2X2, false>), grid, block, 0, stream, q, tiles_m, tiles_n,
                                        kt_per_split);
#undef SDMI_LAUNCH_KIND
  SDMI_HIP_OK(hipGetLastError());
  ps.end();
  if (nsplit > 1) return launch_splitk_reduce(q, nsplit, stream);
  if (q.ln_out) return launch_layernorm(q.out_f32, q.ln_gamma, q.ln_beta, q.ln_out, q.M, q.N, q.ln_eps, stream);
  return 0;
}

}
}
```

### stable-diffusion_amd/csrc/unet.cpp

```cpp
#include "unet.h"

extern "C" char** environ;
#include "prof.h"
#include "split16.h"

#include <math.h>
#include <stdio.h>
#include <string.h>

#include <algorithm>

namespace sdmi {

static bool in_list(const int* v, int n, int x) {
  for (int i = 0; i < n; ++i)
    if (v[i] == x) return true;
  return false;
}

thread_local Tape* g_tape_rec = nullptr;

namespace {
uint64_t sdmi_env_hash() {
  uint64_t h = 1469598103934665603ull;
// ... 245 lines not shown
      if (T.cvt_lo) (void)hipFree(T.cvt_lo);
    }
    return 0;
  });
}

int UNet::set_weight(const char* key, const float* ptr, const int64_t* shape, int ndim, hipStream_t stream) {
  if (int rc = store_.set(key, ptr, shape, ndim, stream)) return rc;
  ++weights_gen_;
  finalized_ = false;
  ctx_valid_ = false;
  drop_timestep_table();
  return 0;
}

int UNet::finalize() {
  if (const WeightSlot* m = store_.missing()) return fail("weight not set: " + m->key);
  if (store_.zero_page()) return -1;
  if (reserve_ctx_cache(8, 77)) return -1;
  {
    SDMI_HIP_OK(hipDeviceSynchronize());
    if (for_each_layer([&](Layer& L) -> int {
      if (L.kind != L_ATTN || full()) return 0;
      const int C = L.cin;
      for (auto& T : L.tb) {
        const int n_[3] = {3 * C, C, 8 * C};
        const f16* w_[3] = {T.wqkv, T.wq2, T.wgg};
        const float* b_[3] = {nullptr, nullptr, T.bgg};
        for (int i = 0; i < 3; ++i) {
          if (store_.alloc((void**)&T.lnf[2 * i], (size_t)n_[i] * sizeof(float)) || store_.alloc((void**)&T.lnf[2 * i + 1], (size_t)n_[i] * sizeof(float)))
            return -1;
          if (launch_ln_fold_prep(w_[i], n_[i], C, C, T.ln[2 * i], T.ln[2 * i + 1], b_[i], T.lnf[2 * i], T.lnf[2 * i + 1], nullptr)) return -1;
        }
        if (ff_tail_supported(C, 32, 32)) {
          if (store_.alloc((void**)&T.lnf_csd, (size_t)16 * C * sizeof(float))) return -1;
          for (int h = 0; h < 4; ++h) {
            SDMI_HIP_OK(hipMemcpyAsync(T.lnf_csd + (size_t)h * 4 * C, T.lnf[4] + (size_t)h * 2 * C, (size_t)2 * C * sizeof(float), hipMemcpyDeviceToDevice, nullptr));
            SDMI_HIP_OK(hipMemcpyAsync(T.lnf_csd + (size_t)h * 4 * C + 2 * C, T.lnf[5] + (size_t)h * 2 * C, (size_t)2 * C * sizeof(float), hipMemcpyDeviceToDevice, nullptr));
          }
        }
      }
      return 0;
    })) return -1;
    if (for_each_layer([&](Layer& L) -> int {
      if (L.kind != L_UP || full() || L.cin % 64 != 0) return 0;
      if (store_.alloc((void**)&L.w_up_phase, (size_t)16 * L.cout * L.cin * sizeof(f16))) return -1;
      return launch_up_phase_weights(L.w16[0], L.w_up_phase, L.cout, L.cin, nullptr);
    })) return -1;
    SDMI_HIP_OK(hipDeviceSynchronize());
    if (for_each_layer([&](Layer& L) -> int {
      if (L.kind != L_RES || L.updown || L.cin == L.cout || !L.f32[5] || !L.f32[6]) return 0;
      std::vector<float> b2((size_t)L.cout), bs((size_t)L.cout);
      SDMI_HIP_OK(hipMemcpy(b2.data(), L.f32[5], b2.size() * sizeof(float), hipMemcpyDeviceToHost));
      SDMI_HIP_OK(hipMemcpy(bs.data(), L.f32[6], bs.size() * sizeof(float), hipMemcpyDeviceToHost));
      for (size_t i = 0; i < b2.size(); ++i) b2[i] += bs[i];
      if (store_.alloc((void**)&L.bias_fold, b2.size() * sizeof(float))) return -1;
      SDMI_HIP_OK(hipMemcpy(L.bias_fold, b2.data(), b2.size() * sizeof(float), hipMemcpyHostToDevice));
      return 0;
    })) return -1;
  }
  ++weights_gen_;
  finalized_ = true;
  return 0;
}

namespace {
// ... 59 lines not shown
  SDMI_CHECK(((h.reserved & PK_NHC_MASK) >> PK_NHC_SHIFT) == num_head_channels_,
             "packed blob was written for num_head_channels " + std::to_string((h.reserved & PK_NHC_MASK) >> PK_NHC_SHIFT) + ", this handle has " +
             std::to_string(num_head_channels_) + ": repack it");
  SDMI_CHECK((h.reserved & ~PK_FULL & ~(7 << 4) & ~PK_NHC_MASK) == ((precise_kv_ ? 1 : 0) | (precise_last_res_ ? 2 : 0) | (precise_1x1_max_ds_ << 8)),
             "packed blob was written with a different precision allocation (context K / V, last ResBlock, 1x1 conv levels)");
  std::vector<std::pair<void**, size_t>> bufs;
  int64_t total = 0;
  packed_layout(&bufs, &total);
  SDMI_CHECK(h.n_buffers == (int32_t)bufs.size() && h.total_bytes == total && bytes >= total, "packed blob truncated or inconsistent");
  int64_t off = (int64_t)round_up((int64_t)sizeof(PackedHeader), PK_ALIGN);
  for (auto& b : bufs) {
    if (store_.alloc(b.first, b.second)) return -1;
    SDMI_HIP_OK(hipMemcpyAsync(*b.first, (const char*)host_buf + off, b.second, hipMemcpyHostToDevice, stream));
    off += (int64_t)round_up((int64_t)b.second, PK_ALIGN);
  }
  SDMI_HIP_OK(hipStreamSynchronize(stream));
  store_.mark_all_set();
  ctx_valid_ = false;
  drop_timestep_table();
  return finalize();
}

struct Fwd : FwdBase {
  UNet* u; int Lctx;
  bool ln_fold_on = false;
  bool ff_tail_on = false;
  bool st_head_on = false;
  bool st_mid_on = false;
  bool st_tail_on = false;
  bool st_mid_ctx_on = false;
  bool ctx1_on = false;
  bool skip_fold_on = false; int skip_fold_max_w = 64;
  std::vector<int>* skip_fold_plan = nullptr;
  bool gn_conv_on = false;
  float* emb_all = nullptr;
  int emb_ld = 0;
  bool emb_caller = false;
  const f16* ctx16 = nullptr;
  const f16* ctx16_lo = nullptr;

  Act res_block(Layer& L, const Act& x0, const Act* x1) {
    const int H = x0.H, W = x0.W, M = B * H * W;
    const int Cin = x0.C + (x1 ? x1->C : 0), Cout = L.cout;
    if (Cin != L.cin) { ok(fail("res block channel mismatch at " + L.prefix)); }
    if (Cin == Cout && x1) ok(fail("identity skip with a concatenated input at " + L.prefix));
    const size_t mark = scratch.off;
    f16* raw = (Cin != Cout) ? S<f16>((size_t)M * Cin) : nullptr;
    const bool p1 = L.p1x1;
    const bool p3 = L.precise3;
    f16* raw_lo = (Cin != Cout && p1) ? S<f16>((size_t)M * Cin) : nullptr;
    float* h = S<float>((size_t)M * Cout);
    Act out = make_act(P<float>((size_t)M * Cout), Cout, H, W, true);
    Act hact = make_act(h, Cout, H, W, true);
    f16* a2 = nullptr;
    int& gn2_applied = u->gn2_applied_;
    gn2_applied = 0;
    const bool ss = u->scale_shift_;
    const float* const film = ss ? emb_all + L.emb_off : nullptr;
    const bool gc1 = gn_conv_on && !ss && !p3 && Cin == Cout && gn_conv3_supported(B, H, W, x0.C, x1 ? x1->C : 0, Cout);
    const bool gc2 = gn_conv_on && !ss && !p3 && gn_conv3_supported(B, H, W, Cout, 0, Cout);
    auto gn_conv = [&](const Act& a0, const Act* a1, const float* gamma, const float* beta, const f16* w, IGemmParams& e) {
      GnConvParams g = GnConvParams();
      g.gn_acc = groupnorm(a0, a1, gamma, beta, 1e-5f, 1, nullptr, nullptr, nullptr, nullptr, nullptr, true);
      g.x0 = a0.p; g.c0 = a0.C; g.x1 = a1 ? a1->p : nullptr; g.c1 = a1 ? a1->C : 0;
      g.gn_gamma = gamma; g.gn_beta = beta; g.gn_eps = 1e-5f; g.w = w; g.epi = e;
      if (!dry && !rc) ok(launch_gn_conv3(g, s));
// ... 43 lines not shown
        residual = out.p;
      }
    }
    if (gc2) {
      IGemmParams p = conv3(nullptr, Cout, H, W, H, W, 1, 0, L.w16[1], Cout);
      p.bias = L.f32[5]; p.residual = residual; p.ldr = Cout; p.out_f32 = out.p; p.ldo = Cout;
      attach_gn_targets(p, out);
      attach_f16_copy(p, out);
      gn_conv(hact, nullptr, L.f32[3], L.f32[4], L.w16[1], p);
    } else {
      f16* a2_lo = nullptr;
      if (p3) { a2 = S<f16>((size_t)M * Cout); a2_lo = S<f16>((size_t)M * Cout); }
      if (ss && !a2) a2 = S<f16>((size_t)M * Cout);
      {
        TapeCaller tc(Tape::R_EMB, emb_caller ? film : nullptr);
        groupnorm(hact, nullptr, L.f32[3], L.f32[4], 1e-5f, 1, a2, nullptr, nullptr, a2_lo, nullptr, false, gn2_applied != 0, film, emb_ld);
      }
      IGemmParams p = conv3(a2, Cout, H, W, H, W, 1, 0, L.w16[1], Cout);
      if (p3) split3(p, a2, a2_lo, Cout);
      p.bias = L.f32[5]; p.residual = residual; p.ldr = Cout; p.out_f32 = out.p; p.ldo = Cout;
      if (tailp.tail_kt) {
        p.tail_a0 = tailp.tail_a0; p.tail_a1 = tailp.tail_a1; p.tail_a2 = tailp.tail_a2; p.tail_c = tailp.tail_c; p.tail_ld = tailp.tail_ld;
        p.tail_w = tailp.tail_w; p.tail_kt = tailp.tail_kt;
        p.bias = L.bias_fold; p.residual = nullptr; p.ldr = 0;
      }
      attach_gn_targets(p, out);
      attach_f16_copy(p, out);
      gemm(p);
    }
    scratch.off = mark;
    return out;
  }

  void context_kv(Layer& L, int d) {
    TBlock& T = L.tb[d];
    const int C = L.cin, Lp = (int)round_up(Lctx, 8);
    const int CD = u->cfg_.context_dim;
    IGemmParams p = dense(ctx16, B * Lctx, CD, T.wkv2, 2 * C, Lctx);
    if (ctx16_lo) split3(p, ctx16, ctx16_lo, CD);
    if (u->full()) {
      const size_t mark = scratch.off;
      float* kv = S<float>((size_t)B * Lctx * 2 * C);
      p.out_f32 = kv; p.ldo = 2 * C;
      gemm(p);
      if (!dry && !rc) ok(launch_split_heads(kv, 2 * C, 0, T.ck, T.ck_lo, 0, B, Lctx, Lp, L.heads, L.dh, s));
      if (!dry && !rc) ok(launch_split_heads(kv, 2 * C, C, T.cvt, T.cvt_lo, 1, B, Lctx, Lp, L.heads, L.dh, s));
      scratch.off = mark;
      return;
    }
    p.mode = EPI_HEADS; p.seg_dst[0] = T.ck; p.seg_dst[1] = T.cvt; p.seg_kind[0] = 0; p.seg_kind[1] = 1;
    p.heads = L.heads; p.dh = L.dh; p.ntok = Lctx; p.ntok_pad = Lp; p.segC = C; p.splitk = 1;
    if (!dry && !rc && Lp != Lctx) {
      hipError_t e = memset_async(T.cvt, 0, (size_t)B * C * Lp * sizeof(f16), s);
      if (e != hipSuccess) ok(fail(std::string("hipMemsetAsync: ") + hipGetErrorString(e)));
    }
    gemm(p);
  }

  Act attn_block_full(Layer& L, const Act& x) {
    const int H = x.H, W = x.W, N = H * W, M = B * N, C = L.cin;
    const int Np = (int)round_up(N, 8), Lp = (int)round_up(Lctx, 8);
    const float scale = 1.0f / sqrtf((float)L.dh);
    const size_t mark = scratch.off;
    f16* a = S<f16>((size_t)M * C); f16* a_lo = S<f16>((size_t)M * C);
    float* t = S<float>((size_t)M * C);
    float* y = S<float>((size_t)M * 8 * C);
    f16* q = S<f16>((size_t)M * C); f16* q_lo = S<f16>((size_t)M * C);
    f16* k = S<f16>((size_t)M * C); f16* k_lo = S<f16>((size_t)M * C);
    f16* vt = S<f16>((size_t)B * C * Np); f16* vt_lo = S<f16>((size_t)B * C * Np);
    f16* gg = S<f16>((size_t)M * 4 * C); f16* gg_lo = S<f16>((size_t)M * 4 * C);
    auto linear = [&](const f16* hi, const f16* lo, int K, const f16* w, int n_out, const float* bias, float* out, bool residual) {
      IGemmParams p = dense1x1(hi, lo, M, K, w, n_out, N, true);
      p.bias = bias; p.out_f32 = out; p.ldo = n_out;
      if (residual) { p.residual = out; p.ldr = n_out; }
      gemm(p);
    };
    auto layernorm = [&](const float* gamma, const float* beta) {
      if (!dry && !rc) ok(launch_layernorm_split(t, gamma, beta, a, a_lo, M, C, 1e-5f, s));
    };
    auto heads = [&](const float* src, int ld, int col0, f16* dst, f16* dst_lo, int kind) {
      if (!dry && !rc) ok(launch_split_heads(src, ld, col0, dst, dst_lo, kind, B, N, Np, L.heads, L.dh, s));
    };
    auto attend = [&](const f16* kk, const f16* kk_lo, const f16* v, const f16* v_lo, int nkv, int nkv_pad) {
      AttnSplitParams p = AttnSplitParams();
      p.q = q; p.q_lo = q_lo; p.k = kk; p.k_lo = kk_lo; p.vt = v; p.vt_lo = v_lo; p.out = a; p.out_lo = a_lo;
      p.BH = B * L.heads; p.heads = L.heads; p.nq = N; p.nkv = nkv; p.nkv_pad = nkv_pad; p.d = L.dh; p.scale = scale;
      if (!dry && !rc) ok(launch_attention_split16(p, s));
    };
    groupnorm(x, nullptr, L.f32[0], L.f32[1], 1e-6f, 0, a, nullptr, nullptr, a_lo, nullptr);
    linear(a, a_lo, C, L.w16[0], C, L.f32[2], t, false);
    for (auto& T : L.tb) {
      layernorm(T.ln[0], T.ln[1]);
      linear(a, a_lo, C, T.wqkv, 3 * C, nullptr, y, false);
      heads(y, 3 * C, 0, q, q_lo, 0); heads(y, 3 * C, C, k, k_lo, 0); heads(y, 3 * C, 2 * C, vt, vt_lo, 1);
      attend(k, k_lo, vt, vt_lo, N, Np);
      linear(a, a_lo, C, T.wo1, C, T.bo1, t, true);
      layernorm(T.ln[2], T.ln[3]);
      if (ctx16) context_kv(L, (int)(&T - L.tb.data()));
      linear(a, a_lo, C, T.wq2, C, nullptr, y, false);
      heads(y, C, 0, q, q_lo, 0);
      attend(T.ck, T.ck_lo, T.cvt, T.cvt_lo, Lctx, Lp);
      linear(a, a_lo, C, T.wo2, C, T.bo2, t, true);
      layernorm(T.ln[4], T.ln[5]);
      linear(a, a_lo, C, T.wgg, 8 * C, T.bgg, y, false);
      if (!dry && !rc) ok(launch_geglu_split(y, M, 4 * C, gg, gg_lo, s));
      linear(gg, gg_lo, 4 * C, T.wff2, C, T.bff2, t, true);
    }
    if (!dry && !rc) ok(launch_cast_f16(t, a, a_lo, (int64_t)M * C, s));
    Act out = make_act(P<float>((size_t)M * C), C, H, W, true);
    {
      IGemmParams p = dense1x1(a, a_lo, M, C, L.w16[1], C, N, true);
      p.bias = L.f32[3]; p.residual = x.p; p.ldr = C; p.out_f32 = out.p; p.ldo = C;
      attach_gn_targets(p, out);
      gemm(p);
    }
    scratch.off = mark;
    return out;
  }

  Act attn_block(Layer& L, const Act& x) {
    if (u->full()) return attn_block_full(L, x);
    const int H = x.H, W = x.W, N = H * W, M = B * N, C = L.cin;
    const int Np = (int)round_up(N, 8), Lp = (int)round_up(Lctx, 8);
    const float scale = 1.0f / sqrtf((float)L.dh);
    const size_t mark = scratch.off;
    f16* xn = S<f16>((size_t)M * C);
    const bool p1 = L.p1x1;
    f16* xn_lo = p1 ? S<f16>((size_t)M * C) : nullptr;
    const bool fold_ln = ln_fold_on && C % 64 == 0 && C <= 1280 && N % 64 == 0 && M % 64 == 0 && M >= u->ln_fold_min_rows_;
    const bool chain_head = st_head_on && fold_ln && p1 && L.tb[0].lnf[0] != nullptr &&
                            st_head_supported(C, M, N, Np, L.heads, L.dh) && dense1x1(nullptr, nullptr, M, C, L.w16[0], C, N, p1).split16;
    long long* gn_stats = nullptr;
    if (chain_head) gn_stats = groupnorm(x, nullptr, L.f32[0], L.f32[1], 1e-6f, 0, nullptr, nullptr, nullptr, nullptr, nullptr, true);
    else groupnorm(x, nullptr, L.f32[0], L.f32[1], 1e-6f, 0, xn, nullptr, nullptr, xn_lo, nullptr);
    float* t = S<float>((size_t)M * C);
    f16* ln = S<f16>((size_t)M * C);
    f16* q = S<f16>((size_t)M * C);
    f16* k = S<f16>((size_t)M * C);
    f16* vt = S<f16>((size_t)B * C * Np);
    f16* ao = S<f16>((size_t)M * C);
    f16* gg = S<f16>((size_t)M * 4 * C);
    float* lnp = fold_ln ? S<float>((size_t)(C / 32) * M * 2) : nullptr;
    auto with_ln = [&](IGemmParams& p, const float* gamma, const float* beta) {
      if (fold_ln) { p.out_f16 = ln; p.f16_scale = gamma; p.lnp_out = lnp; p.splitk = 1; }
      else { p.ln_gamma = gamma; p.ln_beta = beta; p.ln_out = ln; p.ln_eps = 1e-5f; }
    };
    auto fold_in = [&](IGemmParams& p, const float* cs, const float* dn) {
      if (!fold_ln) return;
      p.lnf_part = lnp; p.lnf_npart = C / 32; p.lnf_eps = 1e-5f; p.lnf_cs = cs; p.lnf_d = dn; p.bias = nullptr;
    };
    if (chain_head) {
      TBlock& T = L.tb[0];
      StHeadParams h = StHeadParams();
      h.x = x.p; h.gn_acc = gn_stats; h.gn_gamma = L.f32[0]; h.gn_beta = L.f32[1]; h.gn_eps = 1e-6f;
      h.w_in = L.w16[0]; h.b_in = L.f32[2]; h.t = t; h.ln_gamma = T.ln[0]; h.ln_eps = 1e-5f;
      h.wqkv = T.wqkv; h.lnf_cs = T.lnf[0]; h.lnf_d = T.lnf[1]; h.q = q; h.k = k; h.vt = vt;
      h.M = M; h.B = B; h.ntok = N; h.ntok_pad = Np; h.heads = L.heads; h.dh = L.dh; h.C = C;
      if (!dry && !rc && Np != N) {
        hipError_t e = memset_async(vt, 0, (size_t)B * C * Np * sizeof(f16), s);
        if (e != hipSuccess) ok(fail(std::string("hipMemsetAsync: ") + hipGetErrorString(e)));
      }
      if (!dry && !rc) ok(launch_st_head(h, s));
    } else {
      IGemmParams p = dense1x1(xn, xn_lo, M, C, L.w16[0], C, N, p1);
      p.bias = L.f32[2]; p.out_f32 = t; p.ldo = C;
      with_ln(p, L.tb[0].ln[0], L.tb[0].ln[1]);
      gemm(p);
    }
    const int depth = (int)L.tb.size();
    const bool chain_ff = ff_tail_on && fold_ln && p1 && depth == 1 && L.tb[0].lnf_csd != nullptr && ff_tail_supported(C, M, N) &&
                          dense1x1(nullptr, nullptr, M, C, L.w16[1], C, N, p1).split16;
    const bool chain_tail = chain_ff && st_tail_on;
    for (int d = 0; d < depth; ++d) {
      TBlock& T = L.tb[d];
      if (!(chain_head && d == 0)) {
        IGemmParams p = dense(ln, M, C, T.wqkv, 3 * C, N);
        p.mode = EPI_HEADS; p.seg_dst[0] = q; p.seg_dst[1] = k; p.seg_dst[2] = vt;
        p.seg_kind[0] = 0; p.seg_kind[1] = 0; p.seg_kind[2] = 1;
        p.heads = L.heads; p.dh = L.dh; p.ntok = N; p.ntok_pad = Np; p.segC = C; p.splitk = 1;
        fold_in(p, T.lnf[0], T.lnf[1]);
        if (!dry && !rc && Np != N) {
          hipError_t e = memset_async(vt, 0, (size_t)B * C * Np * sizeof(f16), s);
          if (e != hipSuccess) ok(fail(std::string("hipMemsetAsync: ") + hipGetErrorString(e)));
        }
        gemm(p);
      }
      attention(q, k, vt, ao, L, N, N, Np, scale);
      bool chain_ctx = false;
      const bool chain_mid = st_mid_on && fold_ln && T.lnf[2] != nullptr && st_head_supported(C, M, N, Np, L.heads, L.dh);
      if (chain_mid) {
        StHeadParams h = StHeadParams();
        h.a16 = ao; h.w_in = T.wo1; h.b_in = T.bo1; h.t = t; h.ln_gamma = T.ln[2]; h.ln_eps = 1e-5f;
        h.wqkv = T.wq2; h.lnf_cs = T.lnf[2]; h.lnf_d = T.lnf[3]; h.q = q;
        h.M = M; h.B = B; h.ntok = N; h.ntok_pad = Np; h.heads = L.heads; h.dh = L.dh; h.C = C;
        if (ctx16) context_kv(L, d);
        chain_ctx = st_mid_ctx_on && L.dh == 40 && Lctx <= 128;
        if (chain_ctx) { h.ctx_k = T.ck; h.ctx_vt = T.cvt; h.ctx_nkv = Lctx; h.ctx_nkv_pad = Lp; h.ctx_scale = scale; h.ao_out = ao; }
        if (!dry && !rc) ok(launch_st_mid(h, s));
      } else {
        IGemmParams p = dense(ao, M, C, T.wo1, C, N);
        p.bias = T.bo1; p.residual = t; p.ldr = C; p.out_f32 = t; p.ldo = C;
        with_ln(p, T.ln[2], T.ln[3]);
        gemm(p);
      }
      if (ctx16 && !chain_mid) context_kv(L, d);
      if (chain_mid) {
        if (!chain_ctx) attention(q, T.ck, T.cvt, ao, L, N, Lctx, Lp, scale);
      } else if (ctx1_on && Lctx == 1) {
        if (!dry && !rc) ok(launch_ctx1_broadcast(T.cvt, Lp, ao, B, N, C, s));
      } else {
        IGemmParams p = dense(ln, M, C, T.wq2, C, N);
        p.mode = EPI_HEADS; p.seg_dst[0] = q; p.seg_kind[0] = 0;
        p.heads = L.heads; p.dh = L.dh; p.ntok = N; p.ntok_pad = Np; p.segC = C; p.splitk = 1;
        fold_in(p, T.lnf[2], T.lnf[3]);
        gemm(p);
        attention(q, T.ck, T.cvt, ao, L, N, Lctx, Lp, scale);
      }
      if (!chain_tail) {
        IGemmParams p = dense(ao, M, C, T.wo2, C, N);
        p.bias = T.bo2; p.residual = t; p.ldr = C; p.out_f32 = t; p.ldo = C;
        with_ln(p, T.ln[4], T.ln[5]);
        gemm(p);
      }
      if (chain_ff) break;
      {
        IGemmParams p = dense(ln, M, C, T.wgg, 8 * C, N);
        p.mode = EPI_GEGLU; p.bias = T.bgg; p.out_f16 = gg; p.ldo = 4 * C; p.splitk = 1;
        fold_in(p, T.lnf[4], T.lnf[5]);
        gemm(p);
      }
      {
        IGemmParams p = dense(gg, M, 4 * C, T.wff2, C, N);
        p.bias = T.bff2; p.residual = t; p.ldr = C; p.ldo = C;
        if (d + 1 < depth) {
          p.out_f32 = t;
          with_ln(p, L.tb[d + 1].ln[0], L.tb[d + 1].ln[1]);
        } else {
          p.out_f16 = ln; p.out_lo = xn_lo;
        }
        gemm(p);
      }
    }
    Act out = make_act(P<float>((size_t)M * C), C, H, W, true);
    {
      IGemmParams p = dense1x1(ln, xn_lo, M, C, L.w16[1], C, N, p1);
      p.Hout = H * W;
      p.bias = L.f32[3]; p.residual = x.p; p.ldr = C; p.out_f32 = out.p; p.ldo = C;
      attach_gn_targets(p, out);
      attach_f16_copy(p, out);
      if (chain_ff) {
        TBlock& T = L.tb[0];
// ... 200 lines not shown
  const int mc = cfg_.model_channels;
  const size_t row = (size_t)emb_total_, tmp = (size_t)8 * (mc + 2 * (size_t)te_);
  const size_t need = (size_t)n * row + tmp;
  if (need > emb_tab_floats_) {
    if (emb_tab_) (void)hipFree(emb_tab_);
    emb_tab_ = nullptr; emb_tab_floats_ = 0;
    SDMI_HIP_OK(hipMalloc((void**)&emb_tab_, need * sizeof(float)));
    emb_tab_floats_ = need;
  }
  if ((size_t)n > emb_tab_tcap_) {
    if (emb_tab_tdev_) (void)hipFree(emb_tab_tdev_);
    emb_tab_tdev_ = nullptr; emb_tab_tcap_ = 0;
    SDMI_HIP_OK(hipMalloc((void**)&emb_tab_tdev_, (size_t)n * sizeof(int64_t)));
    emb_tab_tcap_ = (size_t)n;
  }
  std::vector<int64_t> host(t_host, t_host + n);
  emb_tab_src_.swap(host);
  SDMI_HIP_OK(hipMemcpyAsync(emb_tab_tdev_, emb_tab_src_.data(), (size_t)n * sizeof(int64_t), hipMemcpyHostToDevice, stream));
  float* temb = emb_tab_ + (size_t)n * row;
  float* e1 = temb + (size_t)8 * mc;
  float* emb = e1 + (size_t)8 * te_;
  for (int i0 = 0; i0 < n; i0 += 8) {
    const int nb = std::min(8, n - i0);
    int r = launch_timestep_embedding(emb_tab_tdev_ + i0, nullptr, temb, nb, mc, stream);
    if (!r) r = launch_small_linear(temb, mc, te_w0_, te_b0_, e1, te_, nb, te_, mc, 0, stream);
    if (!r) r = launch_small_linear(e1, te_, te_w2_, te_b2_, emb, te_, nb, te_, te_, 1, stream);
    if (!r) r = launch_small_linear(emb, te_, emb_w_, emb_b_, emb_tab_ + (size_t)i0 * row, emb_total_, nb, emb_total_, te_, 1, stream);
    if (r) return r;
  }
  emb_tab_t_ = emb_tab_src_;
  return 0;
}

int UNet::hint_timestep(int64_t t) {
  emb_hint_row_ = -1;
  for (size_t i = 0; i < emb_tab_t_.size(); ++i)
    if (emb_tab_t_[i] == t) { emb_hint_row_ = (int)i; break; }
  return 0;
}

int UNet::run(const float* x, const int64_t* t_i64, const float* t_f32, const float* ctx, float* eps_out, int B, int H,
              int W, int Lctx, void* workspace, int64_t ws_bytes, hipStream_t stream, bool dry, bool ctx_only,
              int64_t* bytes_needed) {
  SDMI_CHECK(dry || finalized_, "sdmi_unet_finalize() has not succeeded yet");
  SDMI_CHECK(B >= 1 && B <= 8, "batch (CFG rows) must be 1..8 per call");
  if (has_ctx()) SDMI_CHECK(H >= 1 && W >= 1 && Lctx >= 1, "bad shape");
  else SDMI_CHECK(H >= 1 && W >= 1 && Lctx == 0 && ctx == nullptr && !ctx_only,
                  "bad shape: this UNet has no cross-attention (AttentionBlocks): pass ctx = NULL and Lctx = 0");
  const int down = 1 << (cfg_.n_levels - 1);
  if (ext_.resblock_updown)
    SDMI_CHECK(H % down == 0 && W % down == 0, "latent H and W must be multiples of " + std::to_string(down) +
               " for resblock_updown (the down ResBlocks' avg_pool2d rounds down, the skip concat needs the sizes back)");
  SDMI_CHECK(H % down == 0 && W % down == 0, "H and W must be divisible by 2^(levels-1) (the UNet's skip concat requires it)");

  const int hint_row = emb_hint_row_;
  if (!dry && !ctx_only) emb_hint_row_ = -1;

  const char* e_rp = getenv("SDMI_REPLAY"); const char* e_rv = getenv("SDMI_REPLAY_VERIFY");
  const bool replay_on = !(e_rp && atoi(e_rp) == 0);
  const bool replay_verify = e_rv && atoi(e_rv) != 0;
  const bool hinted = t_i64 != nullptr && hint_row >= 0 && hint_row < (int)emb_tab_t_.size();
  auto in_ws = [&](const void* p, size_t bytes) {
    return p && (uintptr_t)p < (uintptr_t)workspace + (uint64_t)ws_bytes && (uintptr_t)workspace < (uintptr_t)p + bytes;
  };
  const size_t img = (size_t)B * H * W * sizeof(float);
  const bool tape_ok = replay_on && !dry && !ctx_only && !prof_enabled() && !tune_collecting() && !range_check_enabled() &&
                       workspace != nullptr && (t_i64 || t_f32) && !in_ws(x, img * cfg_.in_channels) && !in_ws(eps_out, img * cfg_.out_channels) &&
                       !in_ws(t_i64 ? (const void*)t_i64 : t_f32, (size_t)B * (t_i64 ? 8 : 4)) &&
                       !in_ws(ctx, (size_t)B * Lctx * cfg_.context_dim * sizeof(float));
  TapeKey tkey;
  uintptr_t caller[Tape::R_COUNT] = {0, 0, 0, 0, 0};
  Tape* rec = nullptr;
  std::unique_ptr<Tape> verify_against;
  if (tape_ok) {
    tkey.B = B; tkey.H = H; tkey.W = W; tkey.Lctx = Lctx; tkey.mode = hinted ? 0 : (t_i64 ? 1 : 2);
    tkey.ws = workspace; tkey.ws_bytes = ws_bytes; tkey.have_ctx = ctx != nullptr;
    tkey.env = sdmi_env_hash() ^ (tune_generation() * 0x9e3779b97f4a7c15ull); tkey.weights_gen = weights_gen_; tkey.ctx_gen = ctx_gen_;
    auto low4 = [](const void* p, int shift) { return (unsigned)((uintptr_t)p & 15) << shift; };
    tkey.align = low4(x, 0) | low4(eps_out, 4) | low4(ctx, 8) | low4(t_i64 ? (const void*)t_i64 : t_f32, 12);
    caller[Tape::R_X] = (uintptr_t)x; caller[Tape::R_OUT] = (uintptr_t)eps_out;
    caller[Tape::R_T] = hinted ? 0 : (t_i64 ? (uintptr_t)t_i64 : (uintptr_t)t_f32);
    caller[Tape::R_CTX] = (uintptr_t)ctx;
    caller[Tape::R_EMB] = hinted ? (uintptr_t)(emb_tab_ + (size_t)hint_row * emb_total_) : 0;
    for (size_t i = 0; i < tapes_.size(); ++i) {
      if (!(tapes_[i].first == tkey)) continue;
      std::unique_ptr<Tape> hit = std::move(tapes_[i].second);
      tapes_.erase(tapes_.begin() + (long)i);
      SDMI_CHECK(finalized_, "sdmi_unet_finalize() has not succeeded yet");
      if (ensure_ctx_cache(B, Lctx, false)) return -1;
// ... 13 lines not shown
  }
  std::unique_ptr<Tape> fresh;
  if (tape_ok) {
    fresh.reset(new Tape());
    memcpy(fresh->caller, caller, sizeof(caller));
    rec = fresh.get();
  }

  Fwd f;
  f.u = this; f.s = stream; f.dry = dry; f.B = B; f.Lctx = Lctx; f.zero = store_.zero(); f.precise_1x1 = precise_1x1_;
  {
    const char* e_fold = getenv("SDMI_LN_FOLD"); const char* e_vec = getenv("SDMI_EPI_VEC");
    f.ln_fold_on = (e_fold ? atoi(e_fold) != 0 : ln_fold_) && !(e_vec && atoi(e_vec) == 0);
    const char* e_ff = getenv("SDMI_FF_TAIL");
    f.ff_tail_on = e_ff ? atoi(e_ff) != 0 : ff_tail_;
    const char* e_sh = getenv("SDMI_ST_HEAD");
    f.st_head_on = e_sh ? atoi(e_sh) != 0 : st_head_;
    const char* e_sm = getenv("SDMI_ST_MID");
    f.st_mid_on = e_sm ? atoi(e_sm) != 0 : st_head_;
    const char* e_st = getenv("SDMI_ST_TAIL");
    f.st_tail_on = e_st ? atoi(e_st) != 0 : ff_tail_;
    const char* e_mc = getenv("SDMI_ST_MID_CTX");
    f.st_mid_ctx_on = e_mc ? atoi(e_mc) != 0 : st_head_;
    const char* e_c1 = getenv("SDMI_CTX1");
    f.ctx1_on = !(e_c1 && atoi(e_c1) == 0);
    const char* e_gc = getenv("SDMI_GN_CONV");
    f.gn_conv_on = e_gc ? atoi(e_gc) != 0 : false;
    const char* e_sf = getenv("SDMI_SKIP_FOLD");
    f.skip_fold_on = e_sf ? atoi(e_sf) != 0 : skip_fold_;
    const char* e_sfw = getenv("SDMI_SKIP_FOLD_MAX_W");
    f.skip_fold_max_w = e_sfw ? atoi(e_sfw) : skip_fold_max_w_;
    skip_fold_plan_.clear();
    f.skip_fold_plan = &skip_fold_plan_;
    if (full()) {
      f.ln_fold_on = f.ff_tail_on = f.st_head_on = f.st_mid_on = f.st_tail_on = f.st_mid_ctx_on = f.gn_conv_on = false;
    }
  }
  int64_t persist_bytes = 0, scratch_bytes = 0;
  for (int pass = 0; pass < 2; ++pass) {
    const bool d = (pass == 0) ? true : false;
    if (pass == 1 && dry) break;
    f.dry = d; f.rc = 0;
    f.n_acts = 0;
    TapeRecGuard tape_guard(d ? nullptr : rec);
    f.plan = fuse_gn_stats_ ? &gn_plan_ : nullptr;
    if (d) gn_plan_.clear();
    f.persist = Arena(); f.scratch = Arena();
    f.persist.dry = f.scratch.dry = d;
    if (!d) {
      SDMI_CHECK(persist_bytes + scratch_bytes <= ws_bytes, "workspace too small: need " +
                 std::to_string(persist_bytes + scratch_bytes) + " bytes, got " + std::to_string(ws_bytes));
      SDMI_CHECK(workspace != nullptr, "workspace is NULL");
      f.persist.base = (char*)workspace; f.persist.cap = (size_t)persist_bytes;
      f.scratch.base = (char*)workspace + persist_bytes; f.scratch.cap = (size_t)scratch_bytes;
      if (ensure_ctx_cache(B, Lctx, ctx_only)) return -1;
    }
    const int mc = cfg_.model_channels;
    if (f.begin_pass((int64_t)12 << 20)) return -1;
    f16* ctx16 = f.P<f16>((size_t)B * Lctx * cfg_.context_dim);
    f16* ctx16_lo = precise_kv_ ? f.P<f16>((size_t)B * Lctx * cfg_.context_dim) : nullptr;
    const bool have_ctx = has_ctx() && ((ctx != nullptr) || d);
    if (!has_ctx()) {
      f.ctx16 = nullptr; f.ctx16_lo = nullptr;
    } else if (have_ctx) {
      if (!d) {
        TapeCaller tc(Tape::R_CTX, ctx);
        int r = launch_cast_f16(ctx, ctx16, ctx16_lo, (int64_t)B * Lctx * cfg_.context_dim, stream);
        if (r) return r;
// ... 108 lines not shown
```

### stable-diffusion_amd/csrc/unet.h

```cpp
#pragma once
#include <stdlib.h>

#include <memory>
#include <string>
#include <utility>
#include <vector>

#include "../../include/sdmi.h"
#include "common.h"
#include "weights.h"

namespace sdmi {

struct Arena {
  char* base = nullptr; size_t cap = 0, off = 0, peak = 0; bool dry = false; bool overflow = false;
  void* alloc(size_t bytes) {
    const size_t a = (off + 255) & ~(size_t)255;
    off = a + bytes;
    peak = std::max(peak, off);
    if (dry) return (void*)(uintptr_t)(a + 4096);
    if (off > cap) { overflow = true; return base; }
    return base + a;
  }
};
// ... 130 lines not shown
      const int cpg = (g.c0 + g.c1) / 32;
      if (dry) {
        const bool f = x0.stats && (!x1 || x1->stats) && x0.id >= 0 && (!x1 || x1->id >= 0);
        if ((int)plan->fused.size() <= idx) plan->fused.resize(idx + 1, 0);
        plan->fused[idx] = f ? 1 : 0;
        if (f) {
          plan->targets[x0.id].push_back({idx, 0, cpg});
          if (x1) plan->targets[x1->id].push_back({idx, g.c0, cpg});
        }
      } else {
        g.skip_stats = (idx < (int)plan->fused.size() && plan->fused[idx]) ? 1 : 0;
      }
    }
    if (!dry && !rc && !(stats_only && g.skip_stats) && !already_applied) ok(launch_groupnorm(g, s));
    return g.acc;
  }
};

enum LayerKind { L_CONV_IN, L_RES, L_ATTN, L_DOWN, L_UP, L_ATTN_LEGACY };

struct TBlock {
  f16* wqkv = nullptr;
  f16* wo1 = nullptr; float* bo1 = nullptr;
  f16* wq2 = nullptr;
  f16* wkv2 = nullptr;
  f16* wo2 = nullptr; float* bo2 = nullptr;
  f16* wgg = nullptr; float* bgg = nullptr;
  f16* wff2 = nullptr; float* bff2 = nullptr;
  float* ln[6] = {nullptr, nullptr, nullptr, nullptr, nullptr, nullptr};
  f16* ck = nullptr; f16* cvt = nullptr;
  f16* ck_lo = nullptr; f16* cvt_lo = nullptr;
  float* lnf[6] = {nullptr, nullptr, nullptr, nullptr, nullptr, nullptr};
  float* lnf_csd = nullptr;
};

struct Layer {
  LayerKind kind = L_RES;
  std::string prefix;
  int cin = 0, cout = 0, heads = 0, dh = 0, emb_off = 0, attn_index = -1;
  int updown = 0;
  bool p1x1 = true, precise3 = false;
  f16* w16[3] = {nullptr, nullptr, nullptr};
  float* w32[1] = {nullptr};
  float* f32[7] = {nullptr, nullptr, nullptr, nullptr, nullptr, nullptr, nullptr};
  float* bias_fold = nullptr;
  f16* w_up_phase = nullptr;
  std::vector<TBlock> tb;
};

class UNet {
 public:
  UNet() = default;
  ~UNet();
  UNet(const UNet&) = delete;
  UNet& operator=(const UNet&) = delete;

  int build(const sdmi_unet_cfg& cfg, int precision = SDMI_PRECISION_MIXED, const sdmi_unet_ext* ext = nullptr, unsigned flags = 0);
  int set_weight(const char* key, const float* ptr, const int64_t* shape, int ndim, hipStream_t stream);
  int finalize();
  int packed_layout(std::vector<std::pair<void**, size_t>>* bufs, int64_t* total) const;
  int export_packed(void* host_buf, int64_t bytes, hipStream_t stream);
  int import_packed(const void* host_buf, int64_t bytes, hipStream_t stream);
  int run(const float* x, const int64_t* t_i64, const float* t_f32, const float* ctx, float* eps_out, int B, int H, int W,
          int Lctx, void* workspace, int64_t ws_bytes, hipStream_t stream, bool dry, bool ctx_only, int64_t* bytes_needed);

  int cache_timesteps(const int64_t* t_host, int n, hipStream_t stream);
  int reserve_ctx_cache(int B, int Lctx);
  int hint_timestep(int64_t t);

  const WeightStore& weights() const { return store_; }

  sdmi_unet_cfg cfg_{};
  sdmi_unet_ext ext_{};
  bool has_ctx() const { return ext_.attention_block == 0; }
  bool scale_shift_ = false;
  int num_head_channels_ = 0;
  int precision_ = SDMI_PRECISION_MIXED;
  bool full() const { return precision_ == SDMI_PRECISION_FULL; }
  int te_ = 0, emb_total_ = 0, n_attn_ = 0;
  bool precise_1x1_ = true;
  bool precise_last_res_ = true;
  int precise_1x1_max_ds_ = 4;
  bool precise_kv_ = true;

 private:
  friend struct Fwd;
  template <class F> int for_each_layer(F&& fn) {
    for (auto& blk : input_blocks_) for (auto& L : blk) if (int r = fn(L)) return r;
    for (auto& L : middle_) if (int r = fn(L)) return r;
    for (auto& blk : output_blocks_) for (auto& L : blk) if (int r = fn(L)) return r;
    return 0;
  }
  int ensure_ctx_cache(int B, int Lctx, bool may_grow);
  GnPlan gn_plan_;
  bool fuse_gn_stats_ = true;
  bool ln_fold_ = true; int ln_fold_min_rows_ = 512;
  bool ff_tail_ = true;
  bool st_head_ = true;
  bool skip_fold_ = true; int skip_fold_max_w_ = 64;
 public:
  std::vector<int> skip_fold_plan_;
 private:

  struct TapeKey {
    int B = 0, H = 0, W = 0, Lctx = 0, mode = 0;
    const void* ws = nullptr; int64_t ws_bytes = 0; bool have_ctx = false;
    uint64_t env = 0, weights_gen = 0, ctx_gen = 0;
    unsigned align = 0;
    bool operator==(const TapeKey& o) const {
      return B == o.B && H == o.H && W == o.W && Lctx == o.Lctx && mode == o.mode && ws == o.ws && ws_bytes == o.ws_bytes &&
             have_ctx == o.have_ctx && env == o.env && weights_gen == o.weights_gen && ctx_gen == o.ctx_gen && align == o.align;
    }
  };
  std::vector<std::pair<TapeKey, std::unique_ptr<Tape>>> tapes_;
  static constexpr size_t kMaxTapes = 12;
  uint64_t weights_gen_ = 0, ctx_gen_ = 0;
  int gn2_applied_ = 0;
 public:
  uint64_t tape_hits_ = 0, tape_records_ = 0;
 private:

  std::vector<std::vector<Layer>> input_blocks_, output_blocks_;
  std::vector<Layer> middle_;
  WeightStore store_;
  float *te_w0_ = nullptr, *te_b0_ = nullptr, *te_w2_ = nullptr, *te_b2_ = nullptr;
  float *emb_w_ = nullptr, *emb_b_ = nullptr;
  float *out_gamma_ = nullptr, *out_beta_ = nullptr, *out_w_ = nullptr, *out_b_ = nullptr;
  bool finalized_ = false;
  int ctx_B_ = 0, ctx_L_ = 0; bool ctx_valid_ = false;
  int64_t ctx_cap_ = 0;
  float* emb_tab_ = nullptr; size_t emb_tab_floats_ = 0;
  int64_t* emb_tab_tdev_ = nullptr; size_t emb_tab_tcap_ = 0;
  std::vector<int64_t> emb_tab_t_;
// ... 7 lines not shown
```

Before: 3.718.

## Fold cross-attention context into precomputed per-sample Q-K and V-O weights

Adds a context-fold path for cross-attention in the wide (C>=1280) transformer blocks. Since the text context is fixed across steps, Wq·K^T and V·Wo are precomputed per sample and head once per context, so cross-attention becomes two GEMMs: one with a segmented-softmax epilogue and one that writes the output projection plus residual. This removes the separate Q projection, attention kernel and out-projection at those layers, but adds per-sample weight strides, a new softmax epilogue, larger folded weights (heads*128 columns), and disables the fused st_mid/st_tail chains where it applies.

```diff
diff --git a/include/sdmi.h b/include/sdmi.h
--- a/include/sdmi.h
+++ b/include/sdmi.h
@@ -64,6 +64,7 @@
 int sdmi_unet_hint_timestep(sdmi_unet* h, int64_t t);
 int sdmi_unet_tape_stats(sdmi_unet* h, int64_t* replayed, int64_t* recorded);
 int sdmi_unet_skip_fold_plan(sdmi_unet* h, int B, int H, int W, int Lctx, int32_t* folded, int cap);
+int sdmi_unet_ctx_fold_plan(sdmi_unet* h, int B, int H, int W, int Lctx, int32_t* folded, int cap);
 
 int sdmi_unet_forward(sdmi_unet* h, const float* x, const int64_t* t_i64, const float* t_f32, const float* ctx,
                       float* eps_out, int B, int H, int W, int Lctx, void* workspace, int64_t workspace_bytes,
@@ -254,6 +255,9 @@
 int sdmi_k_tail_split_range(int nkt, int nsplit, int split, int* begin, int* end);
 int sdmi_k_igemm_up_phase(const sdmi_igemm_desc* d, void* stream);
 int sdmi_k_up_phase_weights(const void* w_packed_f16, void* dst_f16, int N, int Cin, void* stream);
+int sdmi_k_igemm_per_sample(const sdmi_igemm_desc* d, int64_t w_sample_stride, int lnf_sample_stride, int softmax_valid, void* stream);
+int sdmi_k_ctx_fold(const float* kv, const void* wq_f16, const void* wo_f16, void* pk_f16, void* vo_f16, int B, int Lctx, int heads, int dh,
+                    float scale, void* stream);
 int sdmi_k_ff_tail(const sdmi_igemm_desc* proj_out, const void* ln_f16, const float* lnp, float ln_eps, const float* csd,
                    const void* wgg_f16, const void* wff2_f16, const float* bff2, const float* t, void* stream);
 int sdmi_k_st_tail(const sdmi_igemm_desc* proj_out, const void* a_f16, const void* wo_f16, const float* bo, float* t, const float* ln_gamma,
diff --git a/stable-diffusion_amd/_lib.py b/stable-diffusion_amd/_lib.py
--- a/stable-diffusion_amd/_lib.py
+++ b/stable-diffusion_amd/_lib.py
@@ -178,6 +178,9 @@
     'sdmi_k_tail_split_range': (C.c_int, [C.c_int, C.c_int, C.c_int, C.POINTER(C.c_int), C.POINTER(C.c_int)]),
     'sdmi_k_igemm_up_phase': (C.c_int, [C.POINTER(IGemmDesc), c_ptr]),
     'sdmi_k_up_phase_weights': (C.c_int, [c_ptr, c_ptr, C.c_int, C.c_int, c_ptr]),
+    'sdmi_unet_ctx_fold_plan': (C.c_int, [c_ptr, C.c_int, C.c_int, C.c_int, C.c_int, C.POINTER(C.c_int32), C.c_int]),
+    'sdmi_k_igemm_per_sample': (C.c_int, [C.POINTER(IGemmDesc), C.c_int64, C.c_int, C.c_int, c_ptr]),
+    'sdmi_k_ctx_fold': (C.c_int, [c_ptr, c_ptr, c_ptr, c_ptr, c_ptr, C.c_int, C.c_int, C.c_int, C.c_int, C.c_float, c_ptr]),
     'sdmi_tune_lookup': (C.c_int, [C.c_int] * 9 + [C.POINTER(C.c_int), C.POINTER(C.c_int)]),
     'sdmi_unet_skip_fold_plan': (C.c_int, [c_ptr, C.c_int, C.c_int, C.c_int, C.c_int, C.POINTER(C.c_int32), C.c_int]),
     'sdmi_k_ff_tail': (C.c_int, [C.POINTER(IGemmDesc), c_ptr, c_ptr, C.c_float, c_ptr, c_ptr, c_ptr, c_ptr, c_ptr, c_ptr]),
diff --git a/stable-diffusion_amd/build.py b/stable-diffusion_amd/build.py
--- a/stable-diffusion_amd/build.py
+++ b/stable-diffusion_amd/build.py
@@ -9,7 +9,7 @@
 EXTRA = os.environ.get('SDMI_CXXFLAGS', '').split()
 LIB = os.path.join(HERE, os.environ.get('SDMI_LIB_OUT', 'libsdmi.so'))
 OBJ = os.path.join(HERE, 'build' if os.path.basename(LIB) == 'libsdmi.so' else 'build_' + os.path.splitext(os.path.basename(LIB))[0])
-SOURCES = ['igemm_t1.hip', 'igemm_t0.hip', 'igemm_t2.hip', 'igemm_h1.hip', 'igemm_h0.hip', 'igemm_h2.hip', 'igemm.hip', 'conv3halo.hip', 'gemm_split16.hip', 'rowchain.hip', 'gnconv.hip', 'range.hip', 'attn.hip', 'attn_wide.hip', 'attn_split16.hip', 'attn_wide_split16.hip', 'split_ops.hip', 'norm.hip', 'small.hip', 'sampler.hip', 'inpaint.hip', 'patch.hip', 'vit.hip', 'knn.hip', 'textpool.hip', 'rescale.hip', 'weights.cpp', 'unet.cpp', 'vae.cpp', 'clip.cpp', 'bert.cpp', 'api.cpp', 'prof.cpp']
+SOURCES = ['igemm_t1.hip', 'igemm_t0.hip', 'igemm_t2.hip', 'igemm_h1.hip', 'igemm_h0.hip', 'igemm_h2.hip', 'igemm.hip', 'conv3halo.hip', 'gemm_split16.hip', 'rowchain.hip', 'gnconv.hip', 'range.hip', 'attn.hip', 'attn_wide.hip', 'attn_split16.hip', 'attn_wide_split16.hip', 'ctxfold.hip', 'split_ops.hip', 'norm.hip', 'small.hip', 'sampler.hip', 'inpaint.hip', 'patch.hip', 'vit.hip', 'knn.hip', 'textpool.hip', 'rescale.hip', 'weights.cpp', 'unet.cpp', 'vae.cpp', 'clip.cpp', 'bert.cpp', 'api.cpp', 'prof.cpp']
 FLAGS = ['--offload-arch=gfx950', '-O3', '-std=c++17', '-fPIC', '-munsafe-fp-atomics', '-Wall', '-Wno-unused-function',
          '-Wno-unused-variable']
 
diff --git a/stable-diffusion_amd/csrc/api.cpp b/stable-diffusion_amd/csrc/api.cpp
--- a/stable-diffusion_amd/csrc/api.cpp
+++ b/stable-diffusion_amd/csrc/api.cpp
@@ -579,6 +579,22 @@
   IGemmTune t; t.tile = d->tile; t.dma = d->dma;
   return launch_igemm(q, t, (hipStream_t)stream);
 }
+int sdmi_k_igemm_per_sample(const sdmi_igemm_desc* d, int64_t w_sample_stride, int lnf_sample_stride, int softmax_valid, void* stream) {
+  SDMI_CHECK(d, "null descriptor");
+  IGemmParams p = IGemmParams();
+  if (igemm_params_of(d, p)) return -1;
+  p.w_bstride = w_sample_stride; p.lnf_bstride = lnf_sample_stride;
+  if (softmax_valid) { p.mode = EPI_SOFTMAX; p.smx_valid = softmax_valid; }
+  IGemmTune t; t.tile = d->tile; t.dma = d->dma;
+  return launch_igemm(p, t, (hipStream_t)stream);
+}
+int sdmi_k_ctx_fold(const float* kv, const void* wq_f16, const void* wo_f16, void* pk_f16, void* vo_f16, int B, int Lctx, int heads, int dh,
+                    float scale, void* stream) {
+  CtxFoldParams c = CtxFoldParams();
+  c.kv = kv; c.wq = (const f16*)wq_f16; c.wo = (const f16*)wo_f16; c.pk = (f16*)pk_f16; c.vo = (f16*)vo_f16;
+  c.B = B; c.Lctx = Lctx; c.heads = heads; c.dh = dh; c.C = heads * dh; c.scale = scale;
+  return launch_ctx_fold(c, (hipStream_t)stream);
+}
 int sdmi_k_up_phase_weights(const void* w_packed, void* dst, int N, int Cin, void* stream) {
   return launch_up_phase_weights((const f16*)w_packed, (f16*)dst, N, Cin, (hipStream_t)stream);
 }
@@ -596,6 +612,14 @@
   int64_t need = 0;
   if (h->impl.run(nullptr, nullptr, nullptr, nullptr, nullptr, B, H, W, Lctx, nullptr, 0, nullptr, true, false, &need)) return -1;
   const std::vector<int>& plan = h->impl.skip_fold_plan_;
+  for (int i = 0; i < (int)plan.size() && i < cap; ++i) folded[i] = plan[i];
+  return (int)plan.size();
+}
+int sdmi_unet_ctx_fold_plan(sdmi_unet* h, int B, int H, int W, int Lctx, int32_t* folded, int cap) {
+  SDMI_CHECK(h && (folded || cap == 0), "null argument");
+  int64_t need = 0;
+  if (h->impl.run(nullptr, nullptr, nullptr, nullptr, nullptr, B, H, W, Lctx, nullptr, 0, nullptr, true, false, &need)) return -1;
+  const std::vector<int>& plan = h->impl.ctx_fold_plan_;
   for (int i = 0; i < (int)plan.size() && i < cap; ++i) folded[i] = plan[i];
   return (int)plan.size();
 }
diff --git a/stable-diffusion_amd/csrc/common.h b/stable-diffusion_amd/csrc/common.h
--- a/stable-diffusion_amd/csrc/common.h
+++ b/stable-diffusion_amd/csrc/common.h
@@ -71,7 +71,7 @@
 static inline int cdiv(int a, int b) { return (a + b - 1) / b; }
 static inline int64_t round_up(int64_t a, int64_t b) { return (a + b - 1) / b * b; }
 
-enum EpiMode { EPI_PLAIN = 0, EPI_GEGLU = 1, EPI_HEADS = 2 };
+enum EpiMode { EPI_PLAIN = 0, EPI_GEGLU = 1, EPI_HEADS = 2, EPI_SOFTMAX = 3 };
 
 #ifdef SDMI_NT_STORES
 #define SDMI_ST(T, ptr, val) __builtin_nontemporal_store((T)(val), (T*)(ptr))
@@ -177,6 +177,9 @@
   int tail_c = 0, tail_ld = 0;
   const f16* tail_w = nullptr;
   int tail_kt = 0;
+  int64_t w_bstride = 0; int lnf_bstride = 0;
+  int smx_valid = 0;
+  double prof_flops = 0.0;
 };
 __host__ __device__ static inline void tail_split_range(int nkt, int nsplit, int split, int* begin, int* end) {
   *begin = (int)(((long long)split * nkt) / nsplit);
@@ -283,6 +286,15 @@
   int pingpong = 0;
 };
 int launch_attention(const AttnParams& p, hipStream_t stream);
+
+struct CtxFoldParams {
+  const float* kv = nullptr;
+  const f16* wq = nullptr; const f16* wo = nullptr;
+  f16* pk = nullptr; f16* vo = nullptr;
+  int B = 0, Lctx = 0, heads = 0, dh = 0, C = 0;
+  float scale = 1.f;
+};
+int launch_ctx_fold(const CtxFoldParams& p, hipStream_t stream);
 int launch_attention_wide(const AttnParams& p, hipStream_t stream);
 
 struct GroupNormParams {
diff --git a/stable-diffusion_amd/csrc/ctxfold.hip b/stable-diffusion_amd/csrc/ctxfold.hip
--- /dev/null
+++ b/stable-diffusion_amd/csrc/ctxfold.hip
@@ -0,0 +1,84 @@
+#include "common.h"
+#include "prof.h"
+
+namespace sdmi {
+namespace {
+
+__global__ void __launch_bounds__(256) ctx_fold_kernel(const CtxFoldParams p) {
+#if defined(__HIP_DEVICE_COMPILE__)
+  const int lane = threadIdx.x & 63, wave = threadIdx.x >> 6;
+  const int col = lane & 31, hf = lane >> 5;
+  const int which = blockIdx.z & 1;
+  const int g = blockIdx.z >> 1;
+  const int b = g / p.heads, h = g - b * p.heads;
+  const int i0 = blockIdx.y * 32;
+  const int n0 = (blockIdx.x * 4 + wave) * 64;
+  if (n0 >= p.C) return;
+  const int C = p.C, dh = p.dh, S = p.heads * 128;
+  f32x16 acc[2];
+#pragma unroll
+  for (int t = 0; t < 2; ++t)
+#pragma unroll
+    for (int r = 0; r < 16; ++r) acc[t][r] = 0.f;
+  if (i0 < p.Lctx) {
+    const int j = i0 + col;
+    const bool jv = j < p.Lctx;
+    const float* const arow = p.kv + (size_t)(b * p.Lctx + min(j, p.Lctx - 1)) * (size_t)(2 * C) + which * C + h * dh + 4 * hf;
+    for (int d0 = 0; d0 < dh; d0 += 8) {
+      f32x4 a = *(const f32x4*)(arow + d0);
+      if (!jv) a = f32x4{0.f, 0.f, 0.f, 0.f};
+      float bv[2][4];
+      if (which == 0) {
+#pragma unroll
+        for (int t = 0; t < 2; ++t)
+#pragma unroll
+          for (int s = 0; s < 4; ++s) bv[t][s] = (float)p.wq[(size_t)(h * dh + d0 + 4 * hf + s) * C + n0 + t * 32 + col];
+      } else {
+#pragma unroll
+        for (int t = 0; t < 2; ++t) {
+          const f16x4 w = *(const f16x4*)(p.wo + (size_t)(n0 + t * 32 + col) * C + h * dh + d0 + 4 * hf);
+#pragma unroll
+          for (int s = 0; s < 4; ++s) bv[t][s] = (float)w[s];
+        }
+      }
+#pragma unroll
+      for (int s = 0; s < 4; ++s)
+#pragma unroll
+        for (int t = 0; t < 2; ++t) acc[t] = __builtin_amdgcn_mfma_f32_32x32x2f32(a[s], bv[t][s], acc[t], 0, 0, 0);
+    }
+  }
+  if (which == 0) {
+    f16* const dst = p.pk + ((size_t)(b * p.heads + h) * 128 + i0) * (size_t)C + n0 + col;
+#pragma unroll
+    for (int t = 0; t < 2; ++t)
+#pragma unroll
+      for (int r = 0; r < 16; ++r) dst[(size_t)((r & 3) + 8 * (r >> 2) + 4 * hf) * C + t * 32] = (f16)(acc[t][r] * p.scale);
+  } else {
+#pragma unroll
+    for (int t = 0; t < 2; ++t) {
+      f16* const dst = p.vo + ((size_t)b * C + n0 + t * 32 + col) * (size_t)S + h * 128 + i0 + 4 * hf;
+#pragma unroll
+      for (int q = 0; q < 4; ++q)
+        *(f16x4*)(dst + 8 * q) = f16x4{(f16)acc[t][4 * q], (f16)acc[t][4 * q + 1], (f16)acc[t][4 * q + 2], (f16)acc[t][4 * q + 3]};
+    }
+  }
+#endif
+}
+
+}
+
+int launch_ctx_fold(const CtxFoldParams& p, hipStream_t stream) {
+  SDMI_CHECK(p.kv && p.wq && p.wo && p.pk && p.vo, "ctx_fold: null operand");
+  SDMI_CHECK(p.B >= 1 && p.Lctx >= 1 && p.Lctx <= 128 && p.heads >= 1 && p.dh >= 8 && p.dh % 8 == 0 && p.C == p.heads * p.dh && p.C % 64 == 0,
+             "ctx_fold: 1..128 context tokens, head dim % 8 == 0, C = heads * dh a multiple of 64");
+  SDMI_CHECK(((uintptr_t)p.kv & 15) == 0 && ((uintptr_t)p.wo & 7) == 0 && ((uintptr_t)p.vo & 7) == 0, "ctx_fold: kv 16-byte, wo / vo 8-byte aligned");
+  SDMI_CHECK((int64_t)p.B * p.heads * 2 <= 65535, "ctx_fold: too many (sample, head) pairs for one launch");
+  const double macs = 2.0 * p.B * p.heads * 128.0 * p.C * p.dh;
+  ProfScope ps("ctx_fold", 2.0 * macs, (double)p.B * p.Lctx * 2 * p.C * 4.0 + 2.0 * p.C * p.C * 2.0 + 2.0 * p.B * p.heads * 128.0 * p.C * 2.0, stream);
+  SDMI_LAUNCH(ctx_fold_kernel, dim3((unsigned)cdiv(p.C, 256), 4, (unsigned)(p.B * p.heads * 2)), dim3(256), 0, stream, p);
+  SDMI_HIP_OK(hipGetLastError());
+  ps.end();
+  return 0;
+}
+
+}
diff --git a/stable-diffusion_amd/csrc/igemm.hip b/stable-diffusion_amd/csrc/igemm.hip
--- a/stable-diffusion_amd/csrc/igemm.hip
+++ b/stable-diffusion_amd/csrc/igemm.hip
@@ -399,6 +399,11 @@
 };
 static inline bool tile_is_halo(int t) { return t >= 14 && t <= 17; }
 static inline bool tile_tn_even(int t) { return (kTiles[t].bn / kTiles[t].wn / 32) % 2 == 0; }
+static inline bool tile_fits_ctx(const IGemmParams& p, int t) {
+  if (p.mode == EPI_SOFTMAX && (tile_is_halo(t) || kTiles[t].bn % 128 != 0 || kTiles[t].bn / kTiles[t].wn != 64)) return false;
+  if ((p.w_bstride || p.lnf_bstride) && (tile_is_halo(t) || (p.Hout * p.Wout) % kTiles[t].bm != 0)) return false;
+  return true;
+}
 
 static int launch_tile(int tile, const IGemmParams& p, bool dma, int splitk, hipStream_t stream) {
   if (p.tail_kt && !tile_is_halo(tile)) return fail("a GEMM with a 1x1 tail phase was routed to tile " + std::to_string(tile) + ": only the halo-staged conv tiles 14..17 run a tail");
@@ -456,6 +461,12 @@
     if (table_path.size() >= base.size() && table_path.compare(table_path.size() - base.size(), base.size(), base) == 0)
       return table_path.substr(0, table_path.size() - base.size()) + "tune_up_phase_gfx950.txt";
     return table_path + ".up_phase";
+  }
+  static std::string ctx_path_of(const std::string& table_path) {
+    static const std::string base = "tune_gfx950.txt";
+    if (table_path.size() >= base.size() && table_path.compare(table_path.size() - base.size(), base.size(), base) == 0)
+      return table_path.substr(0, table_path.size() - base.size()) + "tune_ctx_fold_gfx950.txt";
+    return table_path + ".ctx_fold";
   }
   void load_file(const std::string& path) {
     FILE* f = fopen(path.c_str(), "r");
@@ -478,6 +489,7 @@
     if (env_int("SDMI_TUNE_DISABLE", 0)) return;
     load_file(default_path());
     load_file(phase_path_of(default_path()));
+    load_file(ctx_path_of(default_path()));
   }
   std::map<TuneKey, TuneChoice>::const_iterator find_entry(TuneKey k) const {
     auto it = table.find(k);
@@ -504,6 +516,7 @@
     if (p.split16 && !split16_tile_supported(t)) continue;
     if (!p.split16 && ((c.ns == 2 && t != 11 && !tile_is_halo(t)) || t == 12 || t == 13)) continue;
     if (p.mode == EPI_GEGLU && !tile_tn_even(t)) continue;
+    if (!tile_fits_ctx(p, t)) continue;
     if (p.lnp_out && (p.M % c.bm || p.N % c.bn || (p.Hout * p.Wout) % c.bm)) continue;
     const long blocks = (long)cdiv(p.M, c.bm) * cdiv(p.N, c.bn);
     if ((long)c.bm > 2L * p.M && c.bm > 64) continue;
@@ -522,7 +535,7 @@
       if (p.splitk != 0) break;
     }
   }
-  if (out.empty()) out.push_back({5, p.splitk > 0 ? p.splitk : 1, 0.0});
+  if (out.empty()) out.push_back({p.mode == EPI_SOFTMAX ? 8 : 5, p.splitk > 0 ? p.splitk : 1, 0.0});
   return out;
 }
 
@@ -574,18 +587,21 @@
   if (n_keys) *n_keys = (int)g_tuner.stats.size();
   ++g_tune_generation;
   const std::string out = (path && *path) ? std::string(path) : Tuner::default_path();
-  bool any_phase = false;
-  for (auto& kv : g_tuner.table) any_phase = any_phase || kv.first.ksize == 2;
-  for (int which = 0; which < (any_phase ? 2 : 1); ++which) {
-    const std::string path_w = which ? Tuner::phase_path_of(out) : out;
+  bool any_phase = false, any_ctx = false;
+  for (auto& kv : g_tuner.table) { any_phase = any_phase || kv.first.ksize == 2; any_ctx = any_ctx || kv.first.mode == EPI_SOFTMAX; }
+  for (int which = 0; which < 3; ++which) {
+    if ((which == 1 && !any_phase) || (which == 2 && !any_ctx)) continue;
+    const std::string path_w = which == 1 ? Tuner::phase_path_of(out) : (which == 2 ? Tuner::ctx_path_of(out) : out);
     FILE* f = fopen(path_w.c_str(), "w");
     if (!f) return fail("cannot write the tuning table to " + path_w);
-    fputs(which ? "# libsdmi igemm tuning table (gfx950), the 2x2 phase convs of the Upsample convs (ksize 2: M = rows of one phase, K = 4 Cin; compared with "
+    fputs(which == 2 ? "# libsdmi igemm tuning table (gfx950), the scores GEMMs of the context-folded cross-attention (mode 3: segment softmax, N = heads * 128, "
+                       "unsplit), measured in situ by tools/tune.py -- M N K ksize stride up mode splitk_req tile splitk us\n"
+          : which ? "# libsdmi igemm tuning table (gfx950), the 2x2 phase convs of the Upsample convs (ksize 2: M = rows of one phase, K = 4 Cin; compared with "
                        "the site's up = 1 row of the main table), measured in situ by tools/tune.py -- M N K ksize stride up mode splitk_req tile splitk us\n"
                      : "# libsdmi igemm tuning table (gfx950), measured in situ by tools/tune.py -- M N K ksize stride up mode splitk_req tile splitk us\n", f);
     for (auto& kv : g_tuner.table) {
       const TuneKey& k = kv.first;
-      if ((k.ksize == 2) != (which == 1)) continue;
+      if ((k.ksize == 2 ? 1 : (k.mode == EPI_SOFTMAX ? 2 : 0)) != which) continue;
       fprintf(f, "%d %d %d %d %d %d %d %d %d %d %.2f", k.M, k.N, k.K, k.ksize, k.stride, k.up, k.mode, k.splitk_req, kv.second.tile,
               kv.second.splitk, kv.second.us);
       if (k.kt) fprintf(f, " %d", k.kt);
@@ -696,6 +712,16 @@
       SDMI_CHECK(p.gn_acc[t] && p.gn_cpg[t] >= 2 && (p.gn_cbase[t] + p.N + p.gn_cpg[t] - 1) / p.gn_cpg[t] <= 32, "bad GroupNorm statistics target");
   }
   if (p.mode == EPI_HEADS) SDMI_CHECK(p.segC > 0 && p.dh > 0 && p.N % p.segC == 0 && p.N / p.segC <= 3, "bad head scatter");
+  if (p.mode == EPI_SOFTMAX)
+    SDMI_CHECK(p.ksize == 1 && !p.split16 && p.N % 128 == 0 && p.smx_valid >= 1 && p.smx_valid <= 128 && p.out_f16 && !p.out_f32 && !p.out_lo &&
+                   p.ldo >= p.N && p.ldo % 4 == 0 && ((uintptr_t)p.out_f16 & 7) == 0 && !p.bias && !p.rowvec && !p.residual && !p.ln_out &&
+                   !p.lnp_out && !p.f16_scale && !p.gn_n && !p.pgn_out && !p.tail_kt && p.splitk <= 1,
+               "segment softmax: a dense unsplit GEMM of N = heads * 128 columns, 1..128 valid columns per segment, an 8-byte aligned fp16 output of "
+               "pitch % 4 == 0 and nothing else in the epilogue");
+  if (p.w_bstride || p.lnf_bstride)
+    SDMI_CHECK(p.ksize == 1 && !p.split16 && p.c1 == 0 && p.c2 == 0 && !p.tail_kt && !p.pgn_out && (p.w_bstride == 0 || (p.w_bstride >= (int64_t)p.N * p.K && p.w_bstride % 8 == 0)) &&
+                   (p.lnf_bstride == 0 || (p.lnf_part && p.lnf_bstride >= p.N)) && (p.mode == EPI_PLAIN || p.mode == EPI_SOFTMAX),
+               "per-sample weights: a dense one-source GEMM on the generic tiles (plain or segment-softmax epilogue), strides of at least one matrix / N");
 
   SDMI_CHECK((int64_t)p.B * p.Hin * p.Win * p.lda0 * 2 + (int64_t)(p.Win + 1) * p.lda0 * 2 < ((int64_t)1 << 31) - 65536 &&
                  (int64_t)p.N * p.K * 2 < ((int64_t)1 << 31) - 65536,
@@ -738,7 +764,7 @@
         const bool split_ok = splitk != 0 ? (sk == splitk && ws_ok)
                                           : (sk == 1 || (ws_ok && nkt / sk >= 4 && (halo || (sk != 5 && sk != 10)) &&
                                                          (!halo || (nkt / 9) % sk == 0)));
-        if (split_ok && (p.mode != EPI_GEGLU || tile_tn_even(tt)) && (!halo || halo_supported(p, kTiles[tt].bm)) &&
+        if (split_ok && (p.mode != EPI_GEGLU || tile_tn_even(tt)) && tile_fits_ctx(p, tt) && (!halo || halo_supported(p, kTiles[tt].bm)) &&
             (!p.split16 || split16_tile_supported(tt)) && (!phase || sk == 1)) {
           tile = tt; splitk = sk;
         }
@@ -755,7 +781,12 @@
     if (p.mode == EPI_GEGLU) tile = 0;
     else if (p.mode == EPI_HEADS) tile = 2;
     else tile = gflop >= 25.0 ? 3 : 5;
-  }
+    if (!tile_fits_ctx(p, tile)) {
+      static const int order[] = {8, 7, 5};
+      for (int t : order) if (tile_fits_ctx(p, t)) { tile = t; break; }
+    }
+  }
+  if (p.mode == EPI_SOFTMAX) splitk = 1;
   if (p.lnp_out) {
     const int hw = p.Hout * p.Wout;
     if (p.M % kTiles[tile].bm || p.N % kTiles[tile].bn || hw % kTiles[tile].bm || (p.split16 && !split16_tile_supported(tile))) tile = 5;
diff --git a/stable-diffusion_amd/csrc/igemm_dev.h b/stable-diffusion_amd/csrc/igemm_dev.h
--- a/stable-diffusion_amd/csrc/igemm_dev.h
+++ b/stable-diffusion_amd/csrc/igemm_dev.h
@@ -134,6 +134,18 @@
   v += __builtin_bit_cast(float, __builtin_amdgcn_update_dpp(0, __builtin_bit_cast(int, v), 0xB1, 0xF, 0xF, true));
   v += __builtin_bit_cast(float, __builtin_amdgcn_update_dpp(0, __builtin_bit_cast(int, v), 0x4E, 0xF, 0xF, true));
   v += __builtin_bit_cast(float, __builtin_amdgcn_update_dpp(0, __builtin_bit_cast(int, v), 0x141, 0xF, 0xF, true));
+  return v;
+}
+__device__ __forceinline__ float sum16_dpp(float v) {
+  v = sum8_dpp(v);
+  v += __builtin_bit_cast(float, __builtin_amdgcn_update_dpp(0, __builtin_bit_cast(int, v), 0x140, 0xF, 0xF, true));
+  return v;
+}
+__device__ __forceinline__ float max16_dpp(float v) {
+  v = fmaxf(v, __builtin_bit_cast(float, __builtin_amdgcn_update_dpp(0, __builtin_bit_cast(int, v), 0xB1, 0xF, 0xF, true)));
+  v = fmaxf(v, __builtin_bit_cast(float, __builtin_amdgcn_update_dpp(0, __builtin_bit_cast(int, v), 0x4E, 0xF, 0xF, true)));
+  v = fmaxf(v, __builtin_bit_cast(float, __builtin_amdgcn_update_dpp(0, __builtin_bit_cast(int, v), 0x141, 0xF, 0xF, true)));
+  v = fmaxf(v, __builtin_bit_cast(float, __builtin_amdgcn_update_dpp(0, __builtin_bit_cast(int, v), 0x140, 0xF, 0xF, true)));
   return v;
 }
 
@@ -248,10 +260,11 @@
     float2* const tab = (float2*)smem;
     if (tid < BM) tab[tid] = float2{lnf_mean, lnf_rstd};
     __syncthreads();
+    const size_t lnf_b = p.lnf_bstride ? (size_t)fast_div_hw(m0, p.magic_hw) * (size_t)p.lnf_bstride : 0;
 #pragma unroll
     for (int j = 0; j < TN; ++j) {
       const int n = min(nw + j * 32 + l31, p.N - 1);
-      const float cs = p.lnf_cs[n], dn = p.lnf_d[n];
+      const float cs = p.lnf_cs[lnf_b + n], dn = p.lnf_d[lnf_b + n];
 #pragma unroll
       for (int i = 0; i < TM; ++i)
 #pragma unroll
@@ -494,6 +507,64 @@
         }
       }
     }
+  } else if (p.mode == EPI_SOFTMAX) {
+    if constexpr (BN % 128 == 0 && WTN == 64 && !PHASE) {
+      constexpr int NW = WARPS_M * WARPS_N;
+      constexpr int NP = SLAB_NPASS<WTN>, RPI = SLAB_RPI<WTN>;
+      static_assert(2 * TM * 32 <= 32 * LSTR && WARPS_N % 2 == 0, "the exchange tables (maxima | sums of the wave's WTM rows) live in the wave's slab region");
+      __syncthreads();
+      float* const wl = slab_base<NW, WTN, LDS_BYTES>(smem, wave);
+      const float* const xl = slab_base<NW, WTN, LDS_BYTES>(smem, wave & ~1);
+      const float* const xr = slab_base<NW, WTN, LDS_BYTES>(smem, wave | 1);
+      const int rl = lane >> 4, c4 = (lane & 15) * 4;
+      const int key0 = ((nw + c4) & 127);
+      const float ninf = -__builtin_inff();
+      f32x4 v[TM][NP];
+      float red[TM][NP];
+#pragma unroll
+      for (int i = 0; i < TM; ++i) {
+        slab_put<TN, LSTR>(wl, acc[i], l31, lg);
+#pragma unroll
+        for (int q = 0; q < NP; ++q) {
+          f32x4 a = *(const f32x4*)(wl + (q * RPI + rl) * LSTR + c4);
+#pragma unroll
+          for (int e = 0; e < 4; ++e) a[e] = (key0 + e < p.smx_valid) ? a[e] : ninf;
+          v[i][q] = a;
+          red[i][q] = max16_dpp(fmaxf(fmaxf(a[0], a[1]), fmaxf(a[2], a[3])));
+        }
+        asm volatile("s_waitcnt lgkmcnt(0)" ::: "memory");
+      }
+#pragma unroll
+      for (int i = 0; i < TM; ++i)
+#pragma unroll
+        for (int q = 0; q < NP; ++q)
+          if ((lane & 15) == 0) wl[i * 32 + q * RPI + rl] = red[i][q];
+      __syncthreads();
+#pragma unroll
+      for (int i = 0; i < TM; ++i)
+#pragma unroll
+        for (int q = 0; q < NP; ++q) {
+          const int wrow = i * 32 + q * RPI + rl;
+          const float m = fmaxf(xl[wrow], xr[wrow]);
+          f32x4 a = v[i][q];
+#pragma unroll
+          for (int e = 0; e < 4; ++e) a[e] = __builtin_amdgcn_exp2f(a[e] - m);
+          v[i][q] = a;
+          red[i][q] = sum16_dpp((a[0] + a[1]) + (a[2] + a[3]));
+          if ((lane & 15) == 0) wl[TM * 32 + wrow] = red[i][q];
+        }
+      __syncthreads();
+#pragma unroll
+      for (int i = 0; i < TM; ++i)
+#pragma unroll
+        for (int q = 0; q < NP; ++q) {
+          const int wrow = i * 32 + q * RPI + rl;
+          const float inv = __builtin_amdgcn_rcpf(xl[TM * 32 + wrow] + xr[TM * 32 + wrow]);
+          const f32x4 a = v[i][q] * inv;
+          const int m = mw + wrow, n = nw + c4;
+          if (m < p.M && n < p.N) SDMI_ST(f16x4, p.out_f16 + (size_t)m * p.ldo + n, (f16x4{(f16)a[0], (f16)a[1], (f16)a[2], (f16)a[3]}));
+        }
+    }
   } else {
     if (unfused_split) {
       float* slab = p.splitk_ws + (size_t)split * p.M * p.N;
diff --git a/stable-diffusion_amd/csrc/igemm_kernel.h b/stable-diffusion_amd/csrc/igemm_kernel.h
--- a/stable-diffusion_amd/csrc/igemm_kernel.h
+++ b/stable-diffusion_amd/csrc/igemm_kernel.h
@@ -130,7 +130,8 @@
   const long long a_shift = (K3 && !UP) ? (long long)(pad_y * p.Win + pad_x) * ld * 2 : 0;
   const char* const srcA0 = (const char*)p.a0 - a_shift; const char* const srcA1 = (const char*)p.a1 - a_shift;
   const char* const srcA2 = (const char*)p.a2 - a_shift;
-  const f16* const w_base = K2 ? p.w + (size_t)split * (size_t)p.N * (size_t)p.K : p.w;
+  const f16* const w_base = K2 ? p.w + (size_t)split * (size_t)p.N * (size_t)p.K
+                               : (p.w_bstride ? p.w + (size_t)fast_div_hw(m0, p.magic_hw) * (size_t)p.w_bstride : p.w);
   const __amdgpu_buffer_rsrc_t rsrc_w = __builtin_amdgcn_make_buffer_rsrc((void*)w_base, 0, OOB, 0x00020000);
   const int pWin = p.Win;
 
@@ -313,6 +314,13 @@
   const int nkt = igemm_nkt(p);
   const int kt_per_split = cdiv(nkt, splitk);
   const int nsplit = cdiv(nkt, kt_per_split);
+  if (p.w_bstride || p.lnf_bstride)
+    SDMI_CHECK((p.Hout * p.Wout) % BM == 0, "per-sample weights: a row tile of " + std::to_string(BM) + " rows would straddle two samples of " +
+                                              std::to_string(p.Hout * p.Wout) + " rows");
+  if (p.mode == EPI_SOFTMAX) {
+    SDMI_CHECK(BN % 128 == 0 && BN / WARPS_N == 64, "segment softmax: the tile's BN must be a multiple of 128 (a 128-column segment lies inside one tile)");
+    SDMI_CHECK(nsplit == 1, "segment softmax: the scores GEMM runs unsplit");
+  }
   IGemmParams q = p;
   q.nkt = nkt;
   q.splitk = nsplit;
@@ -330,7 +338,8 @@
   dim3 grid(tiles_m * tiles_n * (phase ? 4 : nsplit)), block(WARPS_M * WARPS_N * 64);
   static const int by_shape = env_int("SDMI_PROF_SHAPES", 0);
   std::string pname = std::string("igemm_") + std::to_string(BM) + "x" + std::to_string(BN) + "w" +
-                      std::to_string(WARPS_M * WARPS_N) + "s" + std::to_string(NS) + (HALF ? "h" : "") + (phase ? "_up2x2" : "");
+                      std::to_string(WARPS_M * WARPS_N) + "s" + std::to_string(NS) + (HALF ? "h" : "") + (phase ? "_up2x2" : "") +
+                      (p.mode == EPI_SOFTMAX ? "_ctx_scores" : (p.w_bstride ? "_ctx_out" : ""));
   if (by_shape && prof_enabled())
     pname += "_M" + std::to_string(p.M) + "_N" + std::to_string(p.N) + "_K" + std::to_string(p.K) + "_k" +
              std::to_string(p.ksize) + "_m" + std::to_string(p.mode) + "_s" + std::to_string(nsplit);
@@ -341,7 +350,7 @@
   const double cin_alg = p.k_alg > 0 ? (double)p.k_alg : (double)(p.c0 + p.c1 + p.c2);
   const double m_out = phase ? 4.0 * p.M : (double)p.M;
   const double k_ref = phase ? 9.0 * cin_alg : (double)k_alg;
-  ProfScope ps(pname.c_str(), 2.0 * m_out * (double)p.N * k_ref,
+  ProfScope ps(pname.c_str(), p.prof_flops > 0.0 ? p.prof_flops : 2.0 * m_out * (double)p.N * k_ref,
                src_pix * cin_alg * 2.0 + (double)p.N * k_ref * 2.0 + m_out * n_out * out_b +
                    (p.residual ? (double)p.M * p.N * 4.0 : 0.0),
                stream, 2.0 * m_out * (double)p.N * p.K);
diff --git a/stable-diffusion_amd/csrc/unet.cpp b/stable-diffusion_amd/csrc/unet.cpp
--- a/stable-diffusion_amd/csrc/unet.cpp
+++ b/stable-diffusion_amd/csrc/unet.cpp
@@ -301,6 +301,12 @@
             return -1;
           if (launch_ln_fold_prep(w_[i], n_[i], C, C, T.ln[2 * i], T.ln[2 * i + 1], b_[i], T.lnf[2 * i], T.lnf[2 * i + 1], nullptr)) return -1;
         }
+        if (ctx_fold_geom(L)) {
+          const size_t S = (size_t)L.heads * 128;
+          if (store_.alloc((void**)&T.pk, (size_t)kCtxFoldB * S * C * sizeof(f16)) || store_.alloc((void**)&T.vo, (size_t)kCtxFoldB * S * C * sizeof(f16)) ||
+              store_.alloc((void**)&T.pk_cs, (size_t)kCtxFoldB * S * sizeof(float)) || store_.alloc((void**)&T.pk_d, (size_t)kCtxFoldB * S * sizeof(float)))
+            return -1;
+        }
         if (ff_tail_supported(C, 32, 32)) {
           if (store_.alloc((void**)&T.lnf_csd, (size_t)16 * C * sizeof(float))) return -1;
           for (int h = 0; h < 4; ++h) {
@@ -426,6 +432,8 @@
   bool ctx1_on = false;
   bool skip_fold_on = false; int skip_fold_max_w = 64;
   std::vector<int>* skip_fold_plan = nullptr;
+  int ctx_fold = 0, ctx_fold_min_c = 1280;
+  std::vector<int>* ctx_fold_plan = nullptr;
   bool gn_conv_on = false;
   float* emb_all = nullptr;
   int emb_ld = 0;
@@ -535,7 +543,7 @@
     return out;
   }
 
-  void context_kv(Layer& L, int d) {
+  void context_kv(Layer& L, int d, void* kv_buf = nullptr, size_t kv_cap = 0) {
     TBlock& T = L.tb[d];
     const int C = L.cin, Lp = (int)round_up(Lctx, 8);
     const int CD = u->cfg_.context_dim;
@@ -558,7 +566,34 @@
       if (e != hipSuccess) ok(fail(std::string("hipMemsetAsync: ") + hipGetErrorString(e)));
     }
     gemm(p);
-  }
+    if (ctx_fold_shape(L)) {
+      const size_t mark = scratch.off;
+      const size_t kv_need = (size_t)B * Lctx * 2 * C * sizeof(float);
+      float* kv = kv_cap >= kv_need ? (float*)kv_buf : S<float>((size_t)B * Lctx * 2 * C);
+      if (!ctx_builds(L.cin, ctx_fold, ctx_fold_min_c)) { scratch.off = mark; return; }
+      IGemmParams p2 = dense(ctx16, B * Lctx, CD, T.wkv2, 2 * C, Lctx);
+      if (ctx16_lo) split3(p2, ctx16, ctx16_lo, CD);
+      p2.out_f32 = kv; p2.ldo = 2 * C;
+      gemm(p2);
+      if (!dry && !rc) {
+        if (!T.pk || !T.vo || !T.pk_cs || !T.pk_d) { ok(fail("internal: context-fold operands of " + L.prefix + " were not allocated")); return; }
+        CtxFoldParams c = CtxFoldParams();
+        c.kv = kv; c.wq = T.wq2; c.wo = T.wo2; c.pk = T.pk; c.vo = T.vo;
+        c.B = B; c.Lctx = Lctx; c.heads = L.heads; c.dh = L.dh; c.C = C;
+        c.scale = (1.0f / sqrtf((float)L.dh)) * 1.4426950408889634f;
+        ok(launch_ctx_fold(c, s));
+        if (!rc) ok(launch_ln_fold_prep(T.pk, B * L.heads * 128, C, C, T.ln[2], T.ln[3], nullptr, T.pk_cs, T.pk_d, s));
+      }
+      scratch.off = mark;
+    }
+  }
+  bool ctx_fold_shape(const Layer& L) const { return !u->full() && UNet::ctx_fold_geom(L) && B <= UNet::kCtxFoldB && Lctx >= 1 && Lctx <= 128; }
+  bool ctx_folds(const Layer& L, int N, bool chain_mid_ok) const {
+    if (ctx_fold == 0 || !ctx_fold_shape(L) || N % 64 != 0 || (ctx1_on && Lctx == 1)) return false;
+    if (!dry && !ctx16 && !ctx_builds(L.cin, u->ctx_fold_built_knob_, u->ctx_fold_built_min_c_)) return false;
+    return ctx_fold >= 2 || (L.cin >= ctx_fold_min_c && !chain_mid_ok);
+  }
+  static bool ctx_builds(int C, int knob, int min_c) { return knob >= 2 || (knob == 1 && C >= min_c); }
 
   Act attn_block_full(Layer& L, const Act& x) {
     const int H = x.H, W = x.W, N = H * W, M = B * N, C = L.cin;
@@ -622,7 +657,10 @@
   }
 
   Act attn_block(Layer& L, const Act& x) {
-    if (u->full()) return attn_block_full(L, x);
+    if (u->full()) {
+      if (ctx_fold_plan && dry) ctx_fold_plan->insert(ctx_fold_plan->end(), L.tb.size(), 0);
+      return attn_block_full(L, x);
+    }
     const int H = x.H, W = x.W, N = H * W, M = B * N, C = L.cin;
     const int Np = (int)round_up(N, 8), Lp = (int)round_up(Lctx, 8);
     const float scale = 1.0f / sqrtf((float)L.dh);
@@ -673,7 +711,12 @@
     const int depth = (int)L.tb.size();
     const bool chain_ff = ff_tail_on && fold_ln && p1 && depth == 1 && L.tb[0].lnf_csd != nullptr && ff_tail_supported(C, M, N) &&
                           dense1x1(nullptr, nullptr, M, C, L.w16[1], C, N, p1).split16;
-    const bool chain_tail = chain_ff && st_tail_on;
+    const bool chain_mid_ok = st_mid_on && fold_ln && st_head_supported(C, M, N, Np, L.heads, L.dh);
+    const bool fold_ctx = ctx_folds(L, N, chain_mid_ok);
+    if (ctx_fold_plan && dry) ctx_fold_plan->insert(ctx_fold_plan->end(), L.tb.size(), fold_ctx ? 1 : 0);
+    const int SK = L.heads * 128;
+    f16* const pw = gg;
+    const bool chain_tail = chain_ff && st_tail_on && !fold_ctx;
     for (int d = 0; d < depth; ++d) {
       TBlock& T = L.tb[d];
       if (!(chain_head && d == 0)) {
@@ -690,13 +733,13 @@
       }
       attention(q, k, vt, ao, L, N, N, Np, scale);
       bool chain_ctx = false;
-      const bool chain_mid = st_mid_on && fold_ln && T.lnf[2] != nullptr && st_head_supported(C, M, N, Np, L.heads, L.dh);
+      const bool chain_mid = chain_mid_ok && !fold_ctx && T.lnf[2] != nullptr;
       if (chain_mid) {
         StHeadParams h = StHeadParams();
         h.a16 = ao; h.w_in = T.wo1; h.b_in = T.bo1; h.t = t; h.ln_gamma = T.ln[2]; h.ln_eps = 1e-5f;
         h.wqkv = T.wq2; h.lnf_cs = T.lnf[2]; h.lnf_d = T.lnf[3]; h.q = q;
         h.M = M; h.B = B; h.ntok = N; h.ntok_pad = Np; h.heads = L.heads; h.dh = L.dh; h.C = C;
-        if (ctx16) context_kv(L, d);
+        if (ctx16) context_kv(L, d, gg, (size_t)M * 4 * C * sizeof(f16));
         chain_ctx = st_mid_ctx_on && L.dh == 40 && Lctx <= 128;
         if (chain_ctx) { h.ctx_k = T.ck; h.ctx_vt = T.cvt; h.ctx_nkv = Lctx; h.ctx_nkv_pad = Lp; h.ctx_scale = scale; h.ao_out = ao; }
         if (!dry && !rc) ok(launch_st_mid(h, s));
@@ -706,8 +749,24 @@
         with_ln(p, T.ln[2], T.ln[3]);
         gemm(p);
       }
-      if (ctx16 && !chain_mid) context_kv(L, d);
-      if (chain_mid) {
+      if (ctx16 && !chain_mid) context_kv(L, d, gg, (size_t)M * 4 * C * sizeof(f16));
+      if (fold_ctx) {
+        if (!dry && !rc && !(T.pk && T.vo && T.pk_cs && T.pk_d)) ok(fail("internal: context-fold operands of " + L.prefix + " were not allocated"));
+        const double mc2 = 2.0 * M * (double)C * C, mcl = 2.0 * M * (double)C * Lctx;
+        {
+          IGemmParams p = dense(ln, M, C, T.pk, SK, N);
+          p.mode = EPI_SOFTMAX; p.smx_valid = Lctx; p.out_f16 = pw; p.ldo = SK; p.splitk = 1;
+          p.w_bstride = (int64_t)SK * C; p.prof_flops = mc2 + mcl;
+          fold_in(p, T.pk_cs, T.pk_d);
+          if (fold_ln) p.lnf_bstride = SK;
+          gemm(p);
+        }
+        IGemmParams p = dense(pw, M, SK, T.vo, C, N);
+        p.w_bstride = (int64_t)C * SK; p.prof_flops = mcl + mc2;
+        p.bias = T.bo2; p.residual = t; p.ldr = C; p.out_f32 = t; p.ldo = C;
+        with_ln(p, T.ln[4], T.ln[5]);
+        gemm(p);
+      } else if (chain_mid) {
         if (!chain_ctx) attention(q, T.ck, T.cvt, ao, L, N, Lctx, Lp, scale);
       } else if (ctx1_on && Lctx == 1) {
         if (!dry && !rc) ok(launch_ctx1_broadcast(T.cvt, Lp, ao, B, N, C, s));
@@ -719,7 +778,7 @@
         gemm(p);
         attention(q, T.ck, T.cvt, ao, L, N, Lctx, Lp, scale);
       }
-      if (!chain_tail) {
+      if (!chain_tail && !fold_ctx) {
         IGemmParams p = dense(ao, M, C, T.wo2, C, N);
         p.bias = T.bo2; p.residual = t; p.ldr = C; p.out_f32 = t; p.ldo = C;
         with_ln(p, T.ln[4], T.ln[5]);
@@ -986,6 +1045,13 @@
   return 0;
 }
 
+void UNet::note_ctx_fold_built() {
+  const char* e_cf = getenv("SDMI_CTX_FOLD"); const char* e_cfc = getenv("SDMI_CTX_FOLD_MIN_C");
+  const int knob = full() ? 0 : (e_cf ? atoi(e_cf) : ctx_fold_), min_c = e_cfc ? atoi(e_cfc) : ctx_fold_min_c_;
+  if (knob != ctx_fold_built_knob_ || min_c != ctx_fold_built_min_c_) ++ctx_gen_;
+  ctx_fold_built_knob_ = knob; ctx_fold_built_min_c_ = min_c;
+}
+
 int UNet::hint_timestep(int64_t t) {
   emb_hint_row_ = -1;
   for (size_t i = 0; i < emb_tab_t_.size(); ++i)
@@ -1009,6 +1075,7 @@
 
   const int hint_row = emb_hint_row_;
   if (!dry && !ctx_only) emb_hint_row_ = -1;
+  if (!dry && ctx != nullptr && has_ctx()) note_ctx_fold_built();
 
   const char* e_rp = getenv("SDMI_REPLAY"); const char* e_rv = getenv("SDMI_REPLAY_VERIFY");
   const bool replay_on = !(e_rp && atoi(e_rp) == 0);
@@ -1088,8 +1155,15 @@
     f.skip_fold_max_w = e_sfw ? atoi(e_sfw) : skip_fold_max_w_;
     skip_fold_plan_.clear();
     f.skip_fold_plan = &skip_fold_plan_;
+    const char* e_cf = getenv("SDMI_CTX_FOLD");
+    f.ctx_fold = e_cf ? atoi(e_cf) : ctx_fold_;
+    const char* e_cfc = getenv("SDMI_CTX_FOLD_MIN_C");
+    f.ctx_fold_min_c = e_cfc ? atoi(e_cfc) : ctx_fold_min_c_;
+    ctx_fold_plan_.clear();
+    f.ctx_fold_plan = &ctx_fold_plan_;
     if (full()) {
       f.ln_fold_on = f.ff_tail_on = f.st_head_on = f.st_mid_on = f.st_tail_on = f.st_mid_ctx_on = f.gn_conv_on = false;
+      f.ctx_fold = 0;
     }
   }
   int64_t persist_bytes = 0, scratch_bytes = 0;
diff --git a/stable-diffusion_amd/csrc/unet.h b/stable-diffusion_amd/csrc/unet.h
--- a/stable-diffusion_amd/csrc/unet.h
+++ b/stable-diffusion_amd/csrc/unet.h
@@ -186,6 +186,8 @@
   f16* ck_lo = nullptr; f16* cvt_lo = nullptr;
   float* lnf[6] = {nullptr, nullptr, nullptr, nullptr, nullptr, nullptr};
   float* lnf_csd = nullptr;
+  f16* pk = nullptr; f16* vo = nullptr;
+  float* pk_cs = nullptr; float* pk_d = nullptr;
 };
 
 struct Layer {
@@ -252,7 +254,13 @@
   bool ff_tail_ = true;
   bool st_head_ = true;
   bool skip_fold_ = true; int skip_fold_max_w_ = 64;
+  int ctx_fold_ = 1; int ctx_fold_min_c_ = 1280;
+  int ctx_fold_built_knob_ = 0, ctx_fold_built_min_c_ = 0;
+  void note_ctx_fold_built();
  public:
+  static constexpr int kCtxFoldB = 2;
+  static bool ctx_fold_geom(const Layer& L) { return L.kind == L_ATTN && L.cin % 64 == 0 && L.dh % 8 == 0 && L.dh >= 32 && L.heads * L.dh == L.cin; }
+  std::vector<int> ctx_fold_plan_;
   std::vector<int> skip_fold_plan_;
  private:
 
```

Result: no change. 3.738 (median of 6 runs) (+0.6%).
